# QWERTY6191/projected-lmc

Hardware: AMD Instinct MI355X
Metric: MLL+grad iters/sec, n=8192 16-task LMC (higher is better)
Workload: dtype f32; 1 GPU; C3: ProjectedGPModel+ProjectedLMCmll exact training step (PLMC_fast), n=8192 d=8 p=16 q=8 Matern-5/2 fp32; latents sharded q/N per GPU; n_points=8192, n_dim=8, n_tasks=16, n_latents=8, parallelism=latent-shard x1

## Files before the change

include/plmc.h:

```cpp
#ifndef PLMC_H
#define PLMC_H

#include <stddef.h>
#include <stdint.h>

#ifdef __cplusplus
extern "C" {
#endif

enum { PLMC_RBF = 0, PLMC_MATERN12 = 1, PLMC_MATERN32 = 2, PLMC_MATERN52 = 3, PLMC_SPLINE = 4 };

int         plmc_version(void);
int         plmc_block(void);
int64_t     plmc_pad(int64_t n);
int         plmc_max_dim(void);
const char *plmc_last_error(void);
int64_t     plmc_vd_blocks_for(int64_t n_pad, int64_t lda, int elem_bytes);
int64_t     plmc_vd_blocks(int64_t n_pad, int64_t lda);
int64_t     plmc_vd_blocks_keep(int64_t n_pad, int64_t lda);
int64_t     plmc_split_scales_offset(int64_t n_pad, int64_t lda);
int64_t     plmc_grad_scratch_bytes_for(int64_t n_pad, int q, int elem_bytes);
int64_t     plmc_grad_scratch_bytes(int64_t n_pad, int q);
int64_t     plmc_grad_partials_bytes(int64_t n_pad, int q);

int plmc_assemble_f32(int kind, const float *X, int n, int d, const float *ell, const float *oscale,
                      const float *noise, float *A, int64_t lda, int64_t strideA, int q, void *stream);
int plmc_assemble_f64(int kind, const double *X, int n, int d, const double *ell, const double *oscale,
                      const double *noise, double *A, int64_t lda, int64_t strideA, int q, void *stream);

int plmc_write_rhs_f32(const float *rhs, int nrhs, int n, float *A, int64_t lda, int64_t strideA,
                       int c0, int clear_cols, int q, void *stream);
int plmc_write_rhs_f64(const double *rhs, int nrhs, int n, double *A, int64_t lda, int64_t strideA,
                       int c0, int clear_cols, int q, void *stream);

int plmc_assemble_cross_f32(int kind, const float *X, int n, const float *Xs, int ns, int d,
                            const float *ell, const float *oscale, float *Out, int64_t ldo,
                            int64_t strideO, int64_t col0, int64_t n_rows, int q, void *stream);
int plmc_assemble_cross_f64(int kind, const double *X, int n, const double *Xs, int ns, int d,
                            const double *ell, const double *oscale, double *Out, int64_t ldo,
                            int64_t strideO, int64_t col0, int64_t n_rows, int q, void *stream);

#define PLMC_INFO_CHAIN_ABORT 0x7ffffff0
int plmc_potrf_f32(float *A, int64_t n_pad, int64_t lda, int naug, int64_t strideA, float *Vd,
                   double *logdet, int *info, int with_inverse, int q, void *stream);
int plmc_potrf_f64(double *A, int64_t n_pad, int64_t lda, int naug, int64_t strideA, double *Vd,
                   double *logdet, int *info, int with_inverse, int q, void *stream);
int plmc_potrf_ex_f32(float *A, int64_t n_pad, int64_t lda, int naug, int64_t strideA, float *Vd, double *logdet,
                      int *info, int with_inverse, int q, const float *eig_lo, void *stream);
int plmc_potrf_ex_f64(double *A, int64_t n_pad, int64_t lda, int naug, int64_t strideA, double *Vd, double *logdet,
                      int *info, int with_inverse, int q, const double *eig_lo, void *stream);

int plmc_factorize_ex_f32(int kind, const float *X, int n, int d, const float *ell, const float *oscale, const float *noise,
                          float *A, int64_t n_pad, int64_t lda, int naug, int64_t strideA, float *Vd, double *logdet, int *info,
                          int with_inverse, int q, const float *eig_lo, void *stream);
int plmc_factorize_ex_f64(int kind, const double *X, int n, int d, const double *ell, const double *oscale, const double *noise,
                          double *A, int64_t n_pad, int64_t lda, int naug, int64_t strideA, double *Vd, double *logdet, int *info,
                          int with_inverse, int q, const double *eig_lo, void *stream);

int plmc_potrs_aug_f32(float *A, int64_t n_pad, int64_t lda, int naug, int64_t wcol0, int64_t strideA, float *Vd, int q, void *stream);
int plmc_potrs_aug_f64(double *A, int64_t n_pad, int64_t lda, int naug, int64_t wcol0, int64_t strideA, double *Vd, int q, void *stream);
int plmc_potrs_aug_kept_f32(float *A, int64_t n_pad, int64_t lda, int naug, int64_t wcol0, int64_t strideA, float *Vd, int q,
                            const float *eig_lo, void *stream);
int plmc_potrs_aug_kept_f64(double *A, int64_t n_pad, int64_t lda, int naug, int64_t wcol0, int64_t strideA, double *Vd, int q,
                            const double *eig_lo, void *stream);

int plmc_extract_col_f32(const float *A, int64_t n_pad, int64_t lda, int64_t strideA, int c,
                         float *z, double *quad, int q, void *stream);
int plmc_extract_col_f64(const double *A, int64_t n_pad, int64_t lda, int64_t strideA, int c,
                         double *z, double *quad, int q, void *stream);

int plmc_wt_matvec_f32(const float *W, int64_t n_pad, int64_t ldw, int64_t strideW, const float *z,
                       float *alpha, int q, void *stream);
int plmc_wt_matvec_f64(const double *W, int64_t n_pad, int64_t ldw, int64_t strideW, const double *z,
                       double *alpha, int q, void *stream);

int plmc_gemm_tn_f32(int mode, int M, int N, int K, const float *A, int64_t lda, int64_t strideA, const float *B,
                     int64_t ldb, int64_t strideB, float *C, int64_t ldc, int64_t strideC, int batch, void *stream);
int plmc_gemm_tn_f64(int mode, int M, int N, int K, const double *A, int64_t lda, int64_t strideA, const double *B,
                     int64_t ldb, int64_t strideB, double *C, int64_t ldc, int64_t strideC, int batch, void *stream);
#define PLMC_TRI_A_LOWER 1
#define PLMC_TRI_B_LOWER 2
#define PLMC_TRI_A_UPPER 4
#define PLMC_TRI_C_LOWER 8
#define PLMC_TRI_C_ZERO 16
int plmc_gemm_tn_tri_f32(int mode, int tri, int M, int N, int K, const float *A, int64_t lda, int64_t strideA, const float *B,
                         int64_t ldb, int64_t strideB, float *C, int64_t ldc, int64_t strideC, int batch, void *stream);
int plmc_gemm_tn_tri_f64(int mode, int tri, int M, int N, int K, const double *A, int64_t lda, int64_t strideA, const double *B,
                         int64_t ldb, int64_t strideB, double *C, int64_t ldc, int64_t strideC, int batch, void *stream);

int plmc_posterior_moments_f32(const float *A, int64_t n_pad, int64_t lda, int64_t strideA, int ns, float *mean,
                               float *vsq, int q, void *stream);
int plmc_posterior_moments_f64(const double *A, int64_t n_pad, int64_t lda, int64_t strideA, int ns, double *mean,
                               double *vsq, int q, void *stream);
int plmc_mix_posterior_f32(const float *mean_lat, const float *var_lat, const float *Ht, int q, int ns, int p,
                           double eps, float *mean, float *var, void *stream);
int plmc_mix_posterior_f64(const double *mean_lat, const double *var_lat, const double *Ht, int q, int ns, int p,
                           double eps, double *mean, double *var, void *stream);

int plmc_w_diag_f32(const float *W, int64_t n_pad, int64_t ldw, int64_t strideW, float *kinv_diag, int q,
                    void *stream);
int plmc_w_diag_f64(const double *W, int64_t n_pad, int64_t ldw, int64_t strideW, double *kinv_diag, int q,
                    void *stream);

int plmc_kinv_grad_f32(int kind, const float *W, int64_t n_pad, int64_t ldw, int64_t strideW,
                       const float *alpha, const float *X, int n, int d, const float *ell,
                       const float *oscale, double *grad, float *Kinv, int64_t ldk, int64_t strideK,
                       float *kinv_diag, void *partials, int q, void *stream);
int plmc_kinv_grad_f64(int kind, const double *W, int64_t n_pad, int64_t ldw, int64_t strideW,
                       const double *alpha, const double *X, int n, int d, const double *ell,
                       const double *oscale, double *grad, double *Kinv, int64_t ldk, int64_t strideK,
                       double *kinv_diag, void *partials, int q, void *stream);
int plmc_kinv_grad_ex_f32(int kind, const float *W, int64_t n_pad, int64_t ldw, int64_t strideW,
                          const float *alpha, const float *X, int n, int d, const float *ell,
                          const float *oscale, double *grad, float *Kinv, int64_t ldk, int64_t strideK,
                          float *kinv_diag, void *partials, int q, const float *eig_lo, void *stream);
int plmc_kinv_grad_ex_f64(int kind, const double *W, int64_t n_pad, int64_t ldw, int64_t strideW,
                          const double *alpha, const double *X, int n, int d, const double *ell,
                          const double *oscale, double *grad, double *Kinv, int64_t ldk, int64_t strideK,
                          double *kinv_diag, void *partials, int q, const double *eig_lo, void *stream);
int plmc_kinv_grad_vd_f32(int kind, const float *W, int64_t n_pad, int64_t ldw, int64_t strideW,
                          const float *alpha, const float *X, int n, int d, const float *ell,
                          const float *oscale, double *grad, float *Kinv, int64_t ldk, int64_t strideK,
                          float *kinv_diag, void *partials, int q, const float *eig_lo, const float *Vd, void *stream);
int plmc_kinv_grad_vd_f64(int kind, const double *W, int64_t n_pad, int64_t ldw, int64_t strideW,
                          const double *alpha, const double *X, int n, int d, const double *ell,
                          const double *oscale, double *grad, double *Kinv, int64_t ldk, int64_t strideK,
                          double *kinv_diag, void *partials, int q, const double *eig_lo, const double *Vd, void *stream);

int plmc_max_components(void);
int plmc_assemble_add_f32(int kind, const float *X, int n, int d, int ncomp, const float *ell, const float *oscale,
                          const float *noise, float *A, int64_t lda, int64_t strideA, int q, void *stream);
int plmc_assemble_add_f64(int kind, const double *X, int n, int d, int ncomp, const double *ell, const double *oscale,
                          const double *noise, double *A, int64_t lda, int64_t strideA, int q, void *stream);
int plmc_assemble_cross_add_f32(int kind, const float *X, int n, const float *Xs, int ns, int d, int ncomp,
                                const float *ell, const float *oscale, float *Out, int64_t ldo,
                                int64_t strideO, int64_t col0, int64_t n_rows, int q, void *stream);
int plmc_assemble_cross_add_f64(int kind, const double *X, int n, const double *Xs, int ns, int d, int ncomp,
                                const double *ell, const double *oscale, double *Out, int64_t ldo,
                                int64_t strideO, int64_t col0, int64_t n_rows, int q, void *stream);
int plmc_factorize_add_ex_f32(int kind, const float *X, int n, int d, int ncomp, const float *ell, const float *oscale,
                              const float *noise, float *A, int64_t n_pad, int64_t lda, int naug, int64_t strideA, float *Vd,
                              double *logdet, int *info, int with_inverse, int q, const float *eig_lo, void *stream);
int plmc_factorize_add_ex_f64(int kind, const double *X, int n, int d, int ncomp, const double *ell, const double *oscale,
                              const double *noise, double *A, int64_t n_pad, int64_t lda, int naug, int64_t strideA, double *Vd,
                              double *logdet, int *info, int with_inverse, int q, const double *eig_lo, void *stream);
int plmc_kinv_grad_add_vd_f32(int kind, const float *W, int64_t n_pad, int64_t ldw, int64_t strideW,
                              const float *alpha, const float *X, int n, int d, int ncomp, const float *ell,
                              const float *oscale, double *grad, float *Kinv, int64_t ldk, int64_t strideK,
                              float *kinv_diag, void *partials, int q, const float *eig_lo, const float *Vd, void *stream);
int plmc_kinv_grad_add_vd_f64(int kind, const double *W, int64_t n_pad, int64_t ldw, int64_t strideW,
                              const double *alpha, const double *X, int n, int d, int ncomp, const double *ell,
                              const double *oscale, double *grad, double *Kinv, int64_t ldk, int64_t strideK,
                              double *kinv_diag, void *partials, int q, const double *eig_lo, const double *Vd, void *stream);
int plmc_kernel_vjp_add_f32(int kind, const float *X1, int n1, const float *X2, int n2, int d, int ncomp,
                            const float *ell, const float *oscale, const float *G, int64_t ldg,
                            int64_t strideG, double *gX1, double *gEll, double *gOs, int q, void *stream);
int plmc_kernel_vjp_add_f64(int kind, const double *X1, int n1, const double *X2, int n2, int d, int ncomp,
                            const double *ell, const double *oscale, const double *G, int64_t ldg,
                            int64_t strideG, double *gX1, double *gEll, double *gOs, int q, void *stream);

int plmc_sm_max_mixtures(void);
int plmc_sm_max_dim(void);
int64_t plmc_sm_grad_partials_bytes(int64_t n_pad, int q, int nmix, int elem_bytes);
int plmc_assemble_sm_f32(const float *X, int n, int d, int nmix, const float *scales, const float *means, const float *weights,
                         const float *noise, float *A, int64_t lda, int64_t strideA, int q, void *stream);
int plmc_assemble_sm_f64(const double *X, int n, int d, int nmix, const double *scales, const double *means, const double *weights,
                         const double *noise, double *A, int64_t lda, int64_t strideA, int q, void *stream);
int plmc_assemble_cross_sm_f32(const float *X, int n, const float *Xs, int ns, int d, int nmix, const float *scales, const float *means,
                               const float *weights, float *Out, int64_t ldo, int64_t strideO, int64_t col0, int64_t n_rows, int q,
                               void *stream);
int plmc_assemble_cross_sm_f64(const double *X, int n, const double *Xs, int ns, int d, int nmix, const double *scales, const double *means,
                               const double *weights, double *Out, int64_t ldo, int64_t strideO, int64_t col0, int64_t n_rows, int q,
                               void *stream);
int plmc_factorize_sm_ex_f32(const float *X, int n, int d, int nmix, const float *scales, const float *means, const float *weights,
                             const float *noise, float *A, int64_t n_pad, int64_t lda, int naug, int64_t strideA, float *Vd, double *logdet,
                             int *info, int with_inverse, int q, const float *eig_lo, void *stream);
int plmc_factorize_sm_ex_f64(const double *X, int n, int d, int nmix, const double *scales, const double *means, const double *weights,
                             const double *noise, double *A, int64_t n_pad, int64_t lda, int naug, int64_t strideA, double *Vd, double *logdet,
                             int *info, int with_inverse, int q, const double *eig_lo, void *stream);
int plmc_kinv_grad_sm_vd_f32(const float *W, int64_t n_pad, int64_t ldw, int64_t strideW, const float *alpha, const float *X, int n, int d,
                             int nmix, const float *scales, const float *means, const float *weights, double *grad, float *Kinv, int64_t ldk,
                             int64_t strideK, float *kinv_diag, void *partials, int q, const float *eig_lo, const float *Vd, void *stream);
int plmc_kinv_grad_sm_vd_f64(const double *W, int64_t n_pad, int64_t ldw, int64_t strideW, const double *alpha, const double *X, int n, int d,
                             int nmix, const double *scales, const double *means, const double *weights, double *grad, double *Kinv, int64_t ldk,
                             int64_t strideK, double *kinv_diag, void *partials, int q, const double *eig_lo, const double *Vd, void *stream);

int plmc_per_max_dim(void);
int64_t plmc_per_grad_partials_bytes(int64_t n_pad, int q, int elem_bytes);
int plmc_assemble_per_f32(const float *X, int n, int d, const float *ell, const float *period, const float *oscale, const float *noise,
                          float *A, int64_t lda, int64_t strideA, int q, void *stream);
int plmc_assemble_per_f64(const double *X, int n, int d, const double *ell, const double *period, const double *oscale, const double *noise,
                          double *A, int64_t lda, int64_t strideA, int q, void *stream);
int plmc_assemble_cross_per_f32(const float *X, int n, const float *Xs, int ns, int d, const float *ell, const float *period,
                                const float *oscale, float *Out, int64_t ldo, int64_t strideO, int64_t col0, int64_t n_rows, int q,
                                void *stream);
int plmc_assemble_cross_per_f64(const double *X, int n, const double *Xs, int ns, int d, const double *ell, const double *period,
                                const double *oscale, double *Out, int64_t ldo, int64_t strideO, int64_t col0, int64_t n_rows, int q,
                                void *stream);
int plmc_factorize_per_ex_f32(const float *X, int n, int d, const float *ell, const float *period, const float *oscale, const float *noise,
                              float *A, int64_t n_pad, int64_t lda, int naug, int64_t strideA, float *Vd, double *logdet, int *info,
                              int with_inverse, int q, const float *eig_lo, void *stream);
int plmc_factorize_per_ex_f64(const double *X, int n, int d, const double *ell, const double *period, const double *oscale, const double *noise,
                              double *A, int64_t n_pad, int64_t lda, int naug, int64_t strideA, double *Vd, double *logdet, int *info,
                              int with_inverse, int q, const double *eig_lo, void *stream);
int plmc_kinv_grad_per_vd_f32(const float *W, int64_t n_pad, int64_t ldw, int64_t strideW, const float *alpha, const float *X, int n, int d,
                              const float *ell, const float *period, const float *oscale, double *grad, float *Kinv, int64_t ldk,
                              int64_t strideK, float *kinv_diag, void *partials, int q, const float *eig_lo, const float *Vd, void *stream);
int plmc_kinv_grad_per_vd_f64(const double *W, int64_t n_pad, int64_t ldw, int64_t strideW, const double *alpha, const double *X, int n, int d,
                              const double *ell, const double *period, const double *oscale, double *grad, double *Kinv, int64_t ldk,
                              int64_t strideK, double *kinv_diag, void *partials, int q, const double *eig_lo, const double *Vd, void *stream);

int plmc_comm_unique_id(void *id128);
int plmc_comm_init(const void *id128, int rank, int world);
int plmc_comm_world(void);
int plmc_comm_rank(void);
int plmc_comm_allreduce_sum_f32(float *buf, int64_t count, void *stream);
int plmc_comm_allreduce_sum_f64(double *buf, int64_t count, void *stream);
int plmc_comm_destroy(void);

int64_t plmc_lmc_grad_len(int p, int q, int d);
int64_t plmc_lmc_grad_scratch_bytes(int64_t N_pad, int p, int q, int d);
int plmc_lmc_assemble_f32(int kind, const float *X, int n, int d, int p, int q, const float *ell,
                          const float *oscale, const float *B, const float *Sigma, float *A,
                          int64_t lda, void *stream);
int plmc_lmc_assemble_f64(int kind, const double *X, int n, int d, int p, int q, const double *ell,
                          const double *oscale, const double *B, const double *Sigma, double *A,
                          int64_t lda, void *stream);
int plmc_lmc_cross_f32(int kind, const float *X, int n, const float *Xs, int ns, int d, int p, int q,
                       const float *ell, const float *oscale, const float *B, float *Out, int64_t ldo,
                       int64_t col0, int64_t n_rows, void *stream);
int plmc_lmc_cross_f64(int kind, const double *X, int n, const double *Xs, int ns, int d, int p, int q,
                       const double *ell, const double *oscale, const double *B, double *Out,
                       int64_t ldo, int64_t col0, int64_t n_rows, void *stream);
int plmc_lmc_kinv_grad_f32(int kind, const float *W, int64_t N_pad, int64_t ldw, const float *alpha,
                           const float *X, int n, int d, int p, int q, const float *ell,
                           const float *oscale, const float *B, double *grad, void *partials,
                           void *stream);
int plmc_lmc_kinv_grad_f64(int kind, const double *W, int64_t N_pad, int64_t ldw, const double *alpha,
                           const double *X, int n, int d, int p, int q, const double *ell,
                           const double *oscale, const double *B, double *grad, void *partials,
                           void *stream);

int plmc_kernel_vjp_f32(int kind, const float *X1, int n1, const float *X2, int n2, int d,
                        const float *ell, const float *oscale, const float *G, int64_t ldg,
                        int64_t strideG, double *gX1, double *gEll, double *gOs, int q, void *stream);
int plmc_kernel_vjp_f64(int kind, const double *X1, int n1, const double *X2, int n2, int d,
                        const double *ell, const double *oscale, const double *G, int64_t ldg,
                        int64_t strideG, double *gX1, double *gEll, double *gOs, int q, void *stream);

int plmc_qr_max(void);
int plmc_qr_small_f32(const float *A, int m, int n, int64_t lda, float *Q, int64_t ldq, float *R, int64_t ldr,
                      void *stream);
int plmc_qr_small_f64(const double *A, int m, int n, int64_t lda, double *Q, int64_t ldq, double *R, int64_t ldr,
                      void *stream);

int         plmc_prof_enable(int on);
int         plmc_prof_kernels(void);
const char *plmc_prof_name(int id);
int         plmc_prof_collect(double *ms, int64_t *launches, double *flops, double *bytes);
int         plmc_prof_mfma_rate(int kind, void *sink, int64_t sink_bytes, double *tflops);
int         plmc_dev_reload_knobs(void);

#ifdef __cplusplus
}
#endif
#endif
```

projected-lmc_amd/csrc/api.hip:

```cpp
#include <stdlib.h>
#include <mutex>
#include <vector>

#include "api_common.hpp"
#include "../../include/plmc.h"

namespace plmc {
char *err_buf() {
  static thread_local char buf[256] = {0};
  return buf;
}

static const char *kProfNames[PK_COUNT] = {"k_assemble", "k_write_rhs", "k_assemble_cross", "k_diag",   "k_panel",
                                           "k_trail",    "k_wdiag",     "k_trtri_row",      "k_extract_col",
                                           "k_wt_matvec", "k_kinv_grad", "k_reduce_grad", "k_kernel_vjp",
                                           "sweep_total", "k_trail_row", "k_trail_head", "k_gpanel", "k_split_w", "k_posterior_moments"};
struct ProfRec { int id; hipEvent_t a, b; double flops, bytes; };
static unsigned g_prof_mask = 0;
static std::vector<ProfRec> g_recs;
static std::vector<hipEvent_t> g_free;

static hipEvent_t get_event() {
  if (!g_free.empty()) { hipEvent_t e = g_free.back(); g_free.pop_back(); return e; }
  hipEvent_t e;
  if (hipEventCreate(&e) != hipSuccess) return nullptr;
  return e;
}

static std::recursive_mutex g_api_mutex;
void api_lock() { g_api_mutex.lock(); }
void api_unlock() { g_api_mutex.unlock(); }

static Knobs g_knobs;
static bool g_knobs_loaded = false;
static void load_knobs() {
  const char *h = getenv("PLMC_HALF_TILES"), *g = getenv("PLMC_GRP");
  g_knobs.half_tiles = h ? (atoi(h) == 1 ? 1e30 : (double)atoi(h)) : 640.0;
  g_knobs.grp = g ? atoi(g) : 0;
  g_knobs.serial = getenv("PLMC_SERIAL") && atoi(getenv("PLMC_SERIAL")) != 0;
  g_knobs.bulk_lds = getenv("PLMC_BULK_LDS") ? atoi(getenv("PLMC_BULK_LDS")) : -1;
  g_knobs.split = getenv("PLMC_SPLIT") ? atoi(getenv("PLMC_SPLIT")) : 2;
  if (g_knobs.split != 0 && g_knobs.split != 3) g_knobs.split = 2;
  g_knobs.bulk_streams = getenv("PLMC_BULK_STREAMS") ? atoi(getenv("PLMC_BULK_STREAMS")) : 2;
  g_knobs.chain = getenv("PLMC_CHAIN") ? atoi(getenv("PLMC_CHAIN")) : 1;
  g_knobs.chain_nw = getenv("PLMC_CHAIN_NW") ? atoi(getenv("PLMC_CHAIN_NW")) : 0;
  g_knobs.chain_edge = getenv("PLMC_CHAIN_EDGE") ? atoi(getenv("PLMC_CHAIN_EDGE")) : 0;
  g_knobs_loaded = true;
}
const Knobs &knobs() {
  if (!g_knobs_loaded) {
    std::lock_guard<std::recursive_mutex> lk(g_api_mutex);
    if (!g_knobs_loaded) load_knobs();
  }
  return g_knobs;
}

constexpr int SWEEP_CTX = 2;
struct SweepCtx {
  hipStream_t caller = nullptr;
  bool used = false;
  unsigned long long stamp = 0;
  hipStream_t side[2] = {nullptr, nullptr};
  hipEvent_t ev[16] = {nullptr};
};
static SweepCtx g_ctx[64][SWEEP_CTX];
static unsigned long long g_stamp = 0;
static thread_local int t_ctx = 0;
static SweepCtx *cur_ctx() {
  int dev = 0;
  if (hipGetDevice(&dev) != hipSuccess || dev < 0 || dev >= 64) return nullptr;
  return &g_ctx[dev][t_ctx];
}
hipStream_t side_stream(int which) {
  SweepCtx *c = cur_ctx();
  if (!c || which < 0 || which > 1) return nullptr;
  if (!c->side[which]) {
    int lo = 0, hi = 0;
    (void)hipDeviceGetStreamPriorityRange(&lo, &hi);
    if (hipStreamCreateWithPriority(&c->side[which], hipStreamNonBlocking, hi) != hipSuccess) c->side[which] = nullptr;
  }
  return c->side[which];
}
hipEvent_t sync_event(int idx) {
  SweepCtx *c = cur_ctx();
  if (!c) return nullptr;
  hipEvent_t &e = c->ev[idx & 15];
  if (!e && hipEventCreateWithFlags(&e, hipEventDisableTiming) != hipSuccess) e = nullptr;
  return e;
}
void bind_sweep_ctx(hipStream_t caller, int e_prev_idx) {
  int dev = 0;
  if (hipGetDevice(&dev) != hipSuccess || dev < 0 || dev >= 64) { t_ctx = 0; return; }
  SweepCtx *set = g_ctx[dev];
  int pick = -1;
  for (int i = 0; i < SWEEP_CTX; ++i)
    if (set[i].used && set[i].caller == caller) pick = i;
  if (pick < 0) {
    for (int i = 0; i < SWEEP_CTX && pick < 0; ++i)
      if (!set[i].used) pick = i;
    if (pick < 0) {
      pick = 0;
      for (int i = 1; i < SWEEP_CTX; ++i)
        if (set[i].stamp < set[pick].stamp) pick = i;
      if (set[pick].ev[e_prev_idx & 15]) (void)hipStreamWaitEvent(caller, set[pick].ev[e_prev_idx & 15], 0);
    }
    set[pick].caller = caller;
    set[pick].used = true;
  }
  set[pick].stamp = ++g_stamp;
  t_ctx = pick;
}

template <typename T>
__global__ __launch_bounds__(NTHREADS) void k_mfma_rate(T *sink, int iters) {
  using Tr = Traits<T>;
  typename Tr::acc_t acc[16];
#pragma unroll
  for (int i = 0; i < 16; ++i)
#pragma unroll
    for (int r = 0; r < 4; ++r) acc[i][r] = T(0);
  T a[4], b[4];
#pragma unroll
  for (int i = 0; i < 4; ++i) { a[i] = T(1) + T(threadIdx.x & 7) * T(1e-3) + T(i); b[i] = T(0.5) - T(i) * T(1e-3); }
#pragma unroll 1
  for (int it = 0; it < iters; ++it) {
#pragma unroll
    for (int i = 0; i < 16; ++i) acc[i] = Tr::mfma(a[i >> 2], b[i & 3], acc[i]);
  }
  T s = T(0);
#pragma unroll
  for (int i = 0; i < 16; ++i) s += acc[i][0] + acc[i][1] + acc[i][2] + acc[i][3];
  sink[(size_t)blockIdx.x * NTHREADS + threadIdx.x] = s;
}

typedef __bf16 rate_bf16x8 __attribute__((ext_vector_type(8)));
__global__ __launch_bounds__(NTHREADS) void k_mfma_rate_bf16(float *sink, int iters) {
  f32x4 acc[16];
#pragma unroll
  for (int i = 0; i < 16; ++i)
#pragma unroll
    for (int r = 0; r < 4; ++r) acc[i][r] = 0.f;
  rate_bf16x8 a[4], b[4];
#pragma unroll
  for (int i = 0; i < 4; ++i)
#pragma unroll
    for (int j = 0; j < 8; ++j) { a[i][j] = (__bf16)(1.0f + 0.01f * (float)((threadIdx.x + j) & 7) + (float)i); b[i][j] = (__bf16)(0.5f - 0.01f * (float)(i + j)); }
#pragma unroll 1
  for (int it = 0; it < iters; ++it) {
#pragma unroll
    for (int i = 0; i < 16; ++i) acc[i] = __builtin_amdgcn_mfma_f32_16x16x32_bf16(a[i >> 2], b[i & 3], acc[i], 0, 0, 0);
  }
  float s = 0.f;
#pragma unroll
  for (int i = 0; i < 16; ++i) s += acc[i][0] + acc[i][1] + acc[i][2] + acc[i][3];
  sink[(size_t)blockIdx.x * NTHREADS + threadIdx.x] = s;
}

template <typename T, bool BF16 = false> static int mfma_rate_impl(void *sink, int64_t sink_bytes, double *tflops) {
  int dev = 0;
  hipDeviceProp_t prop;
  if (hipGetDevice(&dev) != hipSuccess || hipGetDeviceProperties(&prop, dev) != hipSuccess) return fail("plmc_prof_mfma_rate", "no device");
  const int grid = 4 * prop.multiProcessorCount, iters = 4000;
  if (!sink || !tflops || sink_bytes < (int64_t)grid * NTHREADS * (int64_t)sizeof(T)) return fail("plmc_prof_mfma_rate", "sink too small");
  hipEvent_t e0 = nullptr, e1 = nullptr;
  if (hipEventCreate(&e0) != hipSuccess || hipEventCreate(&e1) != hipSuccess) return fail("plmc_prof_mfma_rate", "event");
  double best = 0.0;
  for (int rep = 0; rep < 3; ++rep) {
    (void)hipEventRecord(e0, nullptr);
    if (BF16) hipLaunchKernelGGL(k_mfma_rate_bf16, dim3(grid), dim3(NTHREADS), 0, nullptr, (float *)sink, iters);
    else hipLaunchKernelGGL(k_mfma_rate<T>, dim3(grid), dim3(NTHREADS), 0, nullptr, (T *)sink, iters);
    (void)hipEventRecord(e1, nullptr);
    float ms = 0.f;
    if (hipEventSynchronize(e1) != hipSuccess || hipEventElapsedTime(&ms, e0, e1) != hipSuccess) break;
    const double fl = (double)grid * (NTHREADS / 64) * (double)iters * 16.0 * 2.0 * 16 * 16 * (BF16 ? 32 : 4);
    if (ms > 0.f && fl / (ms * 1e-3) / 1e12 > best) best = fl / (ms * 1e-3) / 1e12;
  }
  (void)hipEventDestroy(e0);
  (void)hipEventDestroy(e1);
  *tflops = best;
  return launch_status("plmc_prof_mfma_rate");
}

ProfScope::ProfScope(int id, hipStream_t st, double flops, double bytes) : idx_(-1), st_(st) {
  api_lock();
  if (!((g_prof_mask >> id) & 1u) || g_recs.size() >= (1u << 20)) return;
  ProfRec r{id, get_event(), get_event(), flops, bytes};
  if (!r.a || !r.b) return;
  (void)hipEventRecord(r.a, st);
  g_recs.push_back(r);
  idx_ = (long)g_recs.size() - 1;
}
ProfScope::~ProfScope() {
  if (idx_ >= 0) (void)hipEventRecord(g_recs[idx_].b, st_);
  api_unlock();
}
}

extern "C" {
int plmc_version(void) { return 4; }
int plmc_block(void) { return plmc::NB; }
int64_t plmc_pad(int64_t n) { return (n + plmc::NB - 1) / plmc::NB * plmc::NB; }
int plmc_max_dim(void) { return plmc::MAX_DIM; }
const char *plmc_last_error(void) { return plmc::err_buf(); }

int plmc_prof_enable(int on) {
  std::lock_guard<std::recursive_mutex> lk(plmc::g_api_mutex);
  const unsigned prev = plmc::g_prof_mask, all = (1u << plmc::PK_COUNT) - 1u;
  plmc::g_prof_mask = on == 0 ? 0u : (on == 1 ? all : ((unsigned)on >> 1) & all);
  return prev == 0 ? 0 : (prev == all ? 1 : (int)(prev << 1));
}
int plmc_prof_mfma_rate(int kind, void *sink, int64_t sink_bytes, double *tflops) {
  if (kind == 2) return plmc::mfma_rate_impl<float, true>(sink, sink_bytes, tflops);
  return kind ? plmc::mfma_rate_impl<double>(sink, sink_bytes, tflops) : plmc::mfma_rate_impl<float>(sink, sink_bytes, tflops);
}
int plmc_dev_reload_knobs(void) {
  std::lock_guard<std::recursive_mutex> lk(plmc::g_api_mutex);
  plmc::load_knobs();
  return 0;
}
int plmc_prof_kernels(void) { return plmc::PK_COUNT; }
const char *plmc_prof_name(int id) { return (id >= 0 && id < plmc::PK_COUNT) ? plmc::kProfNames[id] : ""; }
int plmc_prof_collect(double *ms, int64_t *launches, double *flops, double *bytes) {
  using namespace plmc;
  std::lock_guard<std::recursive_mutex> lk(g_api_mutex);
  for (int i = 0; i < PK_COUNT; ++i) { ms[i] = 0; launches[i] = 0; flops[i] = 0; bytes[i] = 0; }
  for (auto &r : g_recs) {
    float t = 0.f;
    if (hipEventSynchronize(r.b) == hipSuccess && hipEventElapsedTime(&t, r.a, r.b) == hipSuccess) {
      ms[r.id] += t; launches[r.id] += 1; flops[r.id] += r.flops; bytes[r.id] += r.bytes;
    }
    g_free.push_back(r.a);
    g_free.push_back(r.b);
  }
  g_recs.clear();
  return 0;
}
}
```

projected-lmc_amd/csrc/api_common.hpp:

```cpp
#pragma once
#include <hip/hip_runtime.h>
#include <stdint.h>
#include <stdio.h>
#include <string.h>

#include "gemm_core.hpp"
#include "covariance.hpp"

namespace plmc {

constexpr int MAX_DIM = 32;
constexpr int MAX_COMP = 4;
constexpr int SM_MAX_MIX = 8;
constexpr int SM_MAX_DIM = 8;
constexpr int PER_MAX_DIM = 8;

char *err_buf();

inline int fail(const char *fn, const char *msg) {
  snprintf(err_buf(), 256, "%s: %s", fn, msg);
  return -1;
}

inline int launch_status(const char *fn) {
  hipError_t e = hipGetLastError();
  if (e != hipSuccess) {
    snprintf(err_buf(), 256, "%s: HIP launch failed: %s", fn, hipGetErrorString(e));
    return -2;
  }
  return 0;
}

#define PLMC_REQUIRE(cond, msg) \
  do { if (!(cond)) return plmc::fail(__func__, msg); } while (0)

enum ProfKernel { PK_ASSEMBLE, PK_WRITE_RHS, PK_CROSS, PK_DIAG, PK_PANEL, PK_TRAIL, PK_WDIAG, PK_TRTRI, PK_EXTRACT,
                  PK_WTMV, PK_KINV_GRAD, PK_REDUCE, PK_VJP, PK_SWEEP, PK_TRAIL_ROW, PK_TRAIL_HEAD, PK_GPANEL, PK_SPLIT, PK_POST, PK_COUNT };

struct ProfScope {
  ProfScope(int id, hipStream_t st, double flops, double bytes);
  ~ProfScope();
  long idx_;
  hipStream_t st_;
};

struct Knobs {
  double half_tiles;
  int grp;
  bool serial;
  int bulk_lds;
  int split;
  int bulk_streams;
  int chain;
  int chain_edge;
  int chain_nw;
};
const Knobs &knobs();

enum CovFamily { COV_PLAIN, COV_ADD, COV_SM, COV_PER };
struct CovTable {
  CovFamily family;
  int kind, d, ncomp;
  const void *ell, *second, *oscale;
  static CovTable plain(int kind, int d, const void *ell, const void *oscale) { return {COV_PLAIN, kind, d, 1, ell, nullptr, oscale}; }
  static CovTable add(int kind, int d, int ncomp, const void *ell, const void *oscale) { return {COV_ADD, kind, d, ncomp, ell, nullptr, oscale}; }
  static CovTable sm(int d, int nmix, const void *scales, const void *means, const void *weights) { return {COV_SM, 0, d, nmix, scales, means, weights}; }
  static CovTable per(int d, const void *ell, const void *period, const void *oscale) { return {COV_PER, 0, d, 1, ell, period, oscale}; }
  const char *check() const {
    if (family == COV_ADD) {
      if (kind < 0 || kind > K_MATERN52) return "additive kernels take the stationary kinds only (no spline kernel)";
      if (ncomp < 1 || ncomp > MAX_COMP) return "need 1 <= components <= plmc_max_components()";
    } else if (family == COV_SM) {
      if (ncomp < 1 || ncomp > SM_MAX_MIX) return "need 1 <= mixtures <= plmc_sm_max_mixtures()";
      if (d <= 0 || d > SM_MAX_DIM) return "need 0 < d <= plmc_sm_max_dim()";
    } else if (family == COV_PER) {
      if (d <= 0 || d > PER_MAX_DIM) return "need 0 < d <= plmc_per_max_dim()";
    }
    return (family == COV_SM || family == COV_PER) && !second ? "null pointer" : nullptr;
  }
  CovFamily route() const { return family == COV_ADD && ncomp == 1 ? COV_PLAIN : family; }
  int partials_rows() const { return family == COV_ADD || family == COV_SM ? ncomp : 1; }
};
#define PLMC_REQUIRE_TABLE(t) \
  do { if (const char *why_ = (t).check()) return plmc::fail(__func__, why_); } while (0)

struct AssembleJob {
  CovTable table;
  int n;
  const void *X, *noise;
};
int assemble_rows(const AssembleJob &job, int elem_bytes, void *A, int64_t lda, int64_t strideA, int q, int ib0, int nrows, void *stream,
                  int ncols = -1, int skip = 0);

hipStream_t side_stream(int which = 0);
hipEvent_t sync_event(int idx);
void bind_sweep_ctx(hipStream_t caller, int e_prev_idx);

inline bool aligned16(const void *p) { return (reinterpret_cast<uintptr_t>(p) & 15) == 0; }

}
```

projected-lmc_amd/csrc/kinv_epilogue.inc:

```
  const int lane = tid & 63, wave = tid >> 6;
  const int wm = wave >> 1, wn = wave & 1;
  const T *el = ell + (int64_t)lat * d;
  const T os = oscale ? oscale[lat] : T(1);
  T g_noise = T(0), g_os = T(0);
  auto wave_sum = [&](double v) {
#pragma unroll
    for (int o = 32; o > 0; o >>= 1) v += __shfl_down(v, o, 64);
    return v;
  };
  double *red;

  if constexpr (DCAP <= 8) {
    typedef GradLds<DCAP> L;
    T g[DCAP];
#pragma unroll
    for (int k = 0; k < DCAP; ++k) g[k] = T(0);
    static_assert(L::END <= tile_smem_elems<T>(), "gradient epilogue LDS plan");
    for (int e = tid; e < NB * DCAP; e += NTHREADS) {
      const int r = e / DCAP, k = e % DCAP;
      const int gi = ib * NB + r, gj = jb * NB + r;
      const T inv = k < d ? T(1) / el[k] : T(0);
      smem[L::UI + r * L::LDI + k] = (k < d && gi < n) ? X[(int64_t)gi * d + k] * inv : T(0);
      smem[L::UJ + r * L::LDI + k] = (k < d && gj < n) ? X[(int64_t)gj * d + k] * inv : T(0);
    }
    if (tid < NB) {
      smem[L::AI + tid] = live ? alpha[(int64_t)lat * n_pad + ib * NB + tid] : T(0);
      smem[L::AJ + tid] = live ? alpha[(int64_t)lat * n_pad + jb * NB + tid] : T(0);
    }
    __syncthreads();
    const bool interior = ib < jb && (jb + 1) * NB <= n && !Kinv && !kinv_diag;
#define PLMC_GRAD_TILE(KIND, INT) \
  grad_tile_small<T, DCAP, KIND, INT>(acc, smem, tid, os, ib, jb, n, lat, n_pad, Kinv, ldk, strideK, kinv_diag, g, g_noise, g_os)
    if (interior) {
      if (kind == K_RBF) PLMC_GRAD_TILE(K_RBF, true);
      else if (kind == K_MATERN12) PLMC_GRAD_TILE(K_MATERN12, true);
      else if (kind == K_MATERN32) PLMC_GRAD_TILE(K_MATERN32, true);
      else if (kind == K_MATERN52) PLMC_GRAD_TILE(K_MATERN52, true);
      else PLMC_GRAD_TILE(K_SPLINE, false);
    } else {
      if (kind == K_RBF) PLMC_GRAD_TILE(K_RBF, false);
      else if (kind == K_MATERN12) PLMC_GRAD_TILE(K_MATERN12, false);
      else if (kind == K_MATERN32) PLMC_GRAD_TILE(K_MATERN32, false);
      else if (kind == K_MATERN52) PLMC_GRAD_TILE(K_MATERN52, false);
      else PLMC_GRAD_TILE(K_SPLINE, false);
    }
#undef PLMC_GRAD_TILE
    __syncthreads();
    red = reinterpret_cast<double *>(smem);
#pragma unroll
    for (int k = 0; k < DCAP; ++k) {
      const double s = wave_sum((double)g[k]);
      if (lane == 0) red[wave * GP + k] = s;
    }
  } else {
  constexpr bool KEEP = PLMC_KINV_KEEP;
  constexpr int GH = KEEP ? DCAP : 8;
  constexpr int KD = KEEP ? DCAP : 1;
  const int ldu = d + 1;
  T *ui = smem;
  T *uj = ui + NB * ldu;
  T *ai = uj + NB * ldu;
  T *aj = ai + NB;
  red = reinterpret_cast<double *>(aj + NB);
  static_assert((2 * NB * (MAX_DIM + 1) + 2 * NB) * sizeof(T) + 4 * GP * sizeof(double) <= tile_smem_elems<T>() * sizeof(T),
                "general gradient epilogue LDS plan");
  for (int e = tid; e < NB * d; e += NTHREADS) {
    int r = e / d, k = e % d;
    int gi = ib * NB + r, gj = jb * NB + r;
    T inv = T(1) / el[k];
    ui[r * ldu + k] = gi < n ? X[(int64_t)gi * d + k] * inv : T(0);
    uj[r * ldu + k] = gj < n ? X[(int64_t)gj * d + k] * inv : T(0);
  }
  if (tid < NB) {
    ai[tid] = live ? alpha[(int64_t)lat * n_pad + ib * NB + tid] : T(0);
    aj[tid] = live ? alpha[(int64_t)lat * n_pad + jb * NB + tid] : T(0);
  }
  __syncthreads();
#pragma unroll 1
  for (int k0 = 0; k0 < DCAP; k0 += GH) {
    T g[GH];
#pragma unroll
    for (int k = 0; k < GH; ++k) g[k] = T(0);
    const bool first = k0 == 0;
    if (first || (k0 < d && !SPLINE)) {
#pragma unroll
      for (int mt = 0; mt < 4; ++mt) {
#pragma unroll 1
        for (int r = 0; r < 4; ++r) {
          const int row = tile_row<T>(wm, mt, lane, r);
          const int gi = ib * NB + row;
          T xi[KD];
          const T *uir = ui + row * ldu;
          if constexpr (KEEP) {
#pragma unroll
            for (int k = 0; k < DCAP; ++k) xi[k] = k < d ? uir[k] : T(0);
          }
          const T a_i = ai[row];
#pragma unroll
          for (int nt = 0; nt < 4; ++nt) {
            const int col = tile_col(wn, nt, lane);
            const int gj = jb * NB + col;
            const auto &av = acc.v[mt][nt];
            const T kin = r == 0 ? av[0] : (r == 1 ? av[1] : (r == 2 ? av[2] : av[3]));
            if (first) {
              if (Kinv && gj >= gi) Kinv[(int64_t)lat * strideK + (int64_t)gi * ldk + gj] = kin;
              if (kinv_diag && gi == gj) kinv_diag[(int64_t)lat * n_pad + gi] = kin;
            }
            if (gi < n && gj < n && gj >= gi) {
              const T wij = a_i * aj[col] - kin;
              const T *ujc = uj + col * ldu;
              T df2[KD];
              T r2 = T(0);
              if constexpr (KEEP) {
#pragma unroll
                for (int k = 0; k < DCAP; ++k) {
                  T df = k < d ? xi[k] - ujc[k] : T(0);
                  df2[k] = df * df;
                  r2 += df2[k];
                }
              } else {
#pragma unroll 4
                for (int k = 0; k < d; ++k) { const T df = uir[k] - ujc[k]; r2 += df * df; }
              }
              T val, base;
              if constexpr (SPLINE) {
                val = T(1);
                if constexpr (KEEP) {
#pragma unroll
                  for (int k = 0; k < DCAP; ++k) val *= k < d ? spline_factor(xi[k], ujc[k]) : T(1);
                } else {
#pragma unroll 4
                  for (int k = 0; k < d; ++k) val *= spline_factor(uir[k], ujc[k]);
                }
                base = T(0);
              } else {
                kern_value_base_fast(kind, r2, val, base);
              }
              if (gi == gj) {
                if (first) { g_noise += wij; g_os += wij * val; }
              } else {
                const T c = T(2) * wij * os * base;
                if constexpr (KEEP) {
#pragma unroll
                  for (int k = 0; k < DCAP; ++k) g[k] += c * df2[k];
                } else if constexpr (!SPLINE) {
#pragma unroll
                  for (int k = 0; k < GH; ++k) {
                    const T df = k0 + k < d ? uir[k0 + k] - ujc[k0 + k] : T(0);
                    g[k] += c * df * df;
                  }
                }
                if (first) g_os += T(2) * wij * val;
              }
            }
          }
        }
      }
    }
#pragma unroll
    for (int k = 0; k < GH; ++k) {
      const double s = wave_sum((double)g[k]);
      if (lane == 0) red[wave * GP + k0 + k] = s;
    }
  }
  }

  {
    double s = wave_sum((double)g_noise);
    if (lane == 0) red[wave * GP + MAX_DIM] = s;
    s = wave_sum((double)g_os);
    if (lane == 0) red[wave * GP + MAX_DIM + 1] = s;
  }
  __syncthreads();
  double *out = partials + (((int64_t)lat * m + ib) * m + jb) * GP;
  if (live && tid < GP) {
    const bool used = tid < DCAP || tid >= MAX_DIM;
    out[tid] = used ? red[tid] + red[GP + tid] + red[2 * GP + tid] + red[3 * GP + tid] : 0.0;
  }
```

projected-lmc_amd/csrc/potri_grad.hip:

```cpp
#include <stdlib.h>
#include "api_common.hpp"
#include "covariance.hpp"
#include "bf3_engine.hpp"
#include "vd_layout.hpp"
#include "../../include/plmc.h"

namespace plmc {

constexpr int GP = MAX_DIM + 2;

template <int DCAP> struct GradLds {
  static constexpr int LDI = DCAP + 4;
  static constexpr int UI = 0, UJ = UI + NB * LDI, AI = UJ + NB * LDI, AJ = AI + NB, ACCS = AJ + NB, END = ACCS + 4 * NTHREADS * 4;
};

template <typename T, int DCAP, int KIND, bool INTERIOR>
__device__ __forceinline__ void grad_tile_small(const Acc<T> &acc, T *smem, const int tid, T os, int ib, int jb, int n, int lat, int64_t n_pad,
                                                T *Kinv, int64_t ldk, int64_t strideK, T *kinv_diag, T (&g)[DCAP],
                                                T &g_noise, T &g_os) {
  typedef Pair<T> T2;
  typedef GradLds<DCAP> L;
  constexpr int NP = DCAP / 2;
  const int lane = tid & 63, wave = tid >> 6;
  const int wm = wave >> 1, wn = wave & 1;
  T2 g2[NP];
#pragma unroll
  for (int j = 0; j < NP; ++j) g2[j] = T2{T(0), T(0)};
  T gos = T(0), gnz = T(0);
  T *accs = smem + L::ACCS + tid * 4;
#pragma unroll 1
  for (int mt = 0; mt < 4; ++mt) {
#define PLMC_PARK(M)                                                                                    \
  _Pragma("unroll") for (int nt = 0; nt < 4; ++nt) _Pragma("unroll") for (int r = 0; r < 4; ++r)         \
      accs[nt * NTHREADS * 4 + r] = acc.v[M][nt][r];
    if (mt == 0) { PLMC_PARK(0) } else if (mt == 1) { PLMC_PARK(1) } else if (mt == 2) { PLMC_PARK(2) } else { PLMC_PARK(3) }
#undef PLMC_PARK
#pragma unroll 1
    for (int nt = 0; nt < 4; ++nt) {
      const int col = tile_col(wn, nt, lane);
      const T *ujc = smem + L::UJ + col * L::LDI;
      T2 u2[NP];
#pragma unroll
      for (int j = 0; j < NP; ++j) u2[j] = *reinterpret_cast<const T2 *>(ujc + 2 * j);
      const T a_j = smem[L::AJ + col];
      const int gj = jb * NB + col;
#pragma unroll 1
      for (int r = 0; r < 4; ++r) {
        const int row = tile_row<T>(wm, mt, lane, r);
        const T kin = accs[nt * NTHREADS * 4 + r];
        const T *uir = smem + L::UI + row * L::LDI;
        T2 df[NP];
        T2 r2p = {T(0), T(0)};
#pragma unroll
        for (int j = 0; j < NP; ++j) {
          df[j] = *reinterpret_cast<const T2 *>(uir + 2 * j) - u2[j];
          r2p += df[j] * df[j];
        }
        T val, base;
        if constexpr (KIND == K_SPLINE) {
          val = T(1);
#pragma unroll
          for (int j = 0; j < NP; ++j) {
            const T2 xr = *reinterpret_cast<const T2 *>(uir + 2 * j);
            val *= spline_factor(xr.x, u2[j].x) * spline_factor(xr.y, u2[j].y);
          }
          base = T(0);
        } else {
          kern_value_base_fast(KIND, r2p.x + r2p.y, val, base);
        }
        T w = smem[L::AI + row] * a_j - kin;
        if (!INTERIOR) {
          const int gi = ib * NB + row;
          if (Kinv && gj >= gi) Kinv[(int64_t)lat * strideK + (int64_t)gi * ldk + gj] = kin;
          if (kinv_diag && gi == gj) kinv_diag[(int64_t)lat * n_pad + gi] = kin;
          const bool live = gi < n && gj < n && gj >= gi;
          if (live && gi == gj) gnz += w;
          w = live ? (gj > gi ? T(2) * w : w) : T(0);
        }
        gos += w * val;
        const T c = w * base;
#pragma unroll
        for (int j = 0; j < NP; ++j) g2[j] += (c * df[j]) * df[j];
      }
    }
  }
  const T sc = INTERIOR ? T(2) * os : os;
#pragma unroll
  for (int j = 0; j < NP; ++j) {
    g[2 * j] += sc * g2[j].x;
    g[2 * j + 1] += sc * g2[j].y;
  }
  g_os += INTERIOR ? T(2) * gos : gos;
  g_noise += gnz;
}

template <typename T, int DCAP> constexpr int KG_MIN_WAVES = sizeof(T) == 8 ? 2 : (DCAP <= 8 ? 4 : (DCAP <= 16 ? 2 : 1));

template <typename T, int DCAP, bool SPLINE>
__device__ __forceinline__ void kinv_tile_epilogue(const Acc<T> &acc, T *smem, const int tid, const bool live, int kind, int ib, int jb, int lat,
                                                   int m, int64_t n_pad, const T *__restrict__ alpha, const T *__restrict__ X, int n, int d,
                                                   const T *__restrict__ ell, const T *__restrict__ oscale, T *Kinv, int64_t ldk,
                                                   int64_t strideK, T *kinv_diag, double *__restrict__ partials) {
  if (!live) { n = 0; Kinv = nullptr; kinv_diag = nullptr; }
#define PLMC_KINV_KEEP (DCAP <= 16)
#include "kinv_epilogue.inc"
#undef PLMC_KINV_KEEP
}

#define PLMC_KINV_TILE_PRODUCT                                                                                                                 \
  const int m = (int)(n_pad / NB);                                                                                                             \
  const int lat = (int)blockIdx.x % nlat;                                                                                                      \
  int ib, jb;                                                                                                                                  \
  tri_decode((int)blockIdx.x / nlat, ib, jb);                                                                                                  \
  __shared__ __align__(16) T smem[tile_smem_elems<T>()];                                                                                       \
  const T *Wl = W + (int64_t)lat * strideW + (int64_t)jb * NB * ldw;                                                                           \
  Acc<T> acc;                                                                                                                                  \
  acc.zero();                                                                                                                                  \
  tile_mainloop<T, false, true>(acc, Wl + (int64_t)ib * NB, ldw, Wl + (int64_t)jb * NB, ldw, (int)(n_pad - (int64_t)jb * NB), smem)

template <typename T, int DCAP, bool SPLINE = false>
__global__ __launch_bounds__(NTHREADS, (KG_MIN_WAVES<T, DCAP>)) void k_kinv_grad(int kind, const T *__restrict__ W, int64_t n_pad, int64_t ldw,
                                                         int64_t strideW, const T *__restrict__ alpha,
                                                         const T *__restrict__ X, int n, int d,
                                                         const T *__restrict__ ell, const T *__restrict__ oscale,
                                                         T *Kinv, int64_t ldk, int64_t strideK, T *kinv_diag,
                                                         double *__restrict__ partials, int nlat) {
  PLMC_KINV_TILE_PRODUCT;
  const int tid = threadIdx.x;
  constexpr bool live = true;
#define PLMC_KINV_KEEP (sizeof(T) == 4)
#include "kinv_epilogue.inc"
#undef PLMC_KINV_KEEP
}

#define PLMC_KINV_BF3_TILE_PRODUCT                                                                                                             \
  constexpr int LDS_BYTES = b3_lds_bytes<S>() > 2 * tile_smem_elems<float>() * (int)sizeof(float) ? b3_lds_bytes<S>() : 2 * tile_smem_elems<float>() * (int)sizeof(float); \
  __shared__ __align__(16) unsigned char lds[LDS_BYTES];                                                                                       \
  const int m = (int)(n_pad / NB);                                                                                                             \
  const int SJ = (m + 7) / 8, NSB = SJ * (SJ + 1) / 2;                                                                                         \
  const int w = blockIdx.x, xcd = w & 7, slot = w >> 3;                                                                                        \
  const int gb = xcd + 8 * (slot >> 5), in = slot & 31;                                                                                        \
  if (gb >= nlat * NSB) return;                                                                                                                \
  const int lat = gb / NSB;                                                                                                                    \
  int sa, sj;                                                                                                                                  \
  tri_decode(gb - lat * NSB, sa, sj);                                                                                                          \
  const int ibm = 2 * (4 * sa + (in >> 3)), jb = 8 * sj + (in & 7);                                                                            \
  if (jb >= m || ibm > jb) return;                                                                                                             \
  Acc<float> acc0, acc1;                                                                                                                       \
  acc0.zero();                                                                                                                                 \
  acc1.zero();                                                                                                                                 \
  if (ws_stride > 1) {                                                                                                                         \
    ws_stride = (int64_t)wscale[VD_W_TAG + 1] * NB * NB;                                                                                       \
    wp_lat_stride = 2 * ws_stride;                                                                                                             \
  }                                                                                                                                            \
  const unsigned short *Pl = Wp + (int64_t)lat * wp_lat_stride + b3_index<S>((int64_t)jb * NB, 0, 0, n_pad);                                   \
  b3_mainloop<S, 2, 0, B3NoPre, true>(acc0, acc1, Pl + (int64_t)ibm * NB * 8, n_pad, Pl + (int64_t)jb * NB * 8, n_pad, (int)(n_pad - (int64_t)jb * NB), lds); \
  float ws = wscale[(int64_t)lat * ws_stride];                                                                                                 \
  if (ws_stride > 1 && wscale[(int64_t)lat * ws_stride + VD_W_TAG] != (float)S::NPL) ws = __builtin_nanf("");                                  \
  b3_combine<S>(acc0, acc1, 1.0f / (ws * ws));                                                                                                 \
  const int half = __builtin_amdgcn_readfirstlane((int)threadIdx.x >> 8);                                                                      \
  const int ib = ibm + half

template <class S, int DCAP, bool SPLINE = false>
__global__ __launch_bounds__(B3_NT, 2) void k_kinv_grad_bf3(int kind, int64_t n_pad, const float *__restrict__ alpha, const float *__restrict__ X, int n,
                                                            int d, const float *__restrict__ ell, const float *__restrict__ oscale, float *Kinv,
                                                            int64_t ldk, int64_t strideK, float *kinv_diag, double *__restrict__ partials, int nlat,
                                                            const unsigned short *__restrict__ Wp, const float *__restrict__ wscale,
                                                            int64_t wp_lat_stride, int64_t ws_stride) {
  PLMC_KINV_BF3_TILE_PRODUCT;
  kinv_tile_epilogue<float, DCAP, SPLINE>(acc0, reinterpret_cast<float *>(lds) + half * tile_smem_elems<float>(), (int)threadIdx.x & 255, ib <= jb, kind,
                                          ib, jb, lat, m, n_pad, alpha, X, n, d, ell, oscale, Kinv, ldk, strideK, kinv_diag, partials);
}


template <typename T, CovFamily F, int DC>
__device__ __forceinline__ void kinv_tile_epilogue_add(const Acc<T> &acc, T *smem, const int tid, const bool live, int kind, int ncomp, int ib, int jb,
                                                       int lat, int m, int64_t n_pad, const T *__restrict__ alpha, const T *__restrict__ X, int n, int d,
                                                       const T *__restrict__ ell, const T *__restrict__ oscale, T *Kinv, int64_t ldk,
                                                       int64_t strideK, T *kinv_diag, double *__restrict__ partials, const T *__restrict__ means) {
  if (!live) { n = 0; Kinv = nullptr; kinv_diag = nullptr; }
#include "kinv_epilogue_table.inc"
}

template <typename T, CovFamily F, int DC = 0>
__global__ __launch_bounds__(NTHREADS, (sizeof(T) == 8 && (F == COV_SM || (F == COV_PER && DC > 1)) ? 1 : 2)) void k_kinv_grad_add(int kind, int ncomp, const T *__restrict__ W, int64_t n_pad, int64_t ldw,
                                                                int64_t strideW, const T *__restrict__ alpha, const T *__restrict__ X, int n, int d,
                                                                const T *__restrict__ ell, const T *__restrict__ oscale, T *Kinv, int64_t ldk,
                                                                int64_t strideK, T *kinv_diag, double *__restrict__ partials, int nlat,
                                                                const T *__restrict__ means) {
  PLMC_KINV_TILE_PRODUCT;
  const int tid = threadIdx.x;
  constexpr bool live = true;
#include "kinv_epilogue_table.inc"
}

template <class S, CovFamily F, int DC = 0>
__global__ __launch_bounds__(B3_NT, 2) void k_kinv_grad_add_bf3(int kind, int ncomp, int64_t n_pad, const float *__restrict__ alpha,
                                                                const float *__restrict__ X, int n, int d, const float *__restrict__ ell,
                                                                const float *__restrict__ oscale, float *Kinv, int64_t ldk, int64_t strideK,
                                                                float *kinv_diag, double *__restrict__ partials, int nlat,
                                                                const unsigned short *__restrict__ Wp, const float *__restrict__ wscale,
                                                                int64_t wp_lat_stride, int64_t ws_stride, const float *__restrict__ means) {
  PLMC_KINV_BF3_TILE_PRODUCT;
  kinv_tile_epilogue_add<float, F, DC>(acc0, reinterpret_cast<float *>(lds) + half * tile_smem_elems<float>(), (int)threadIdx.x & 255, ib <= jb, kind, ncomp,
                                       ib, jb, lat, m, n_pad, alpha, X, n, d, ell, oscale, Kinv, ldk, strideK, kinv_diag, partials, means);
}

constexpr int RED_NT = 1024;
#define PLMC_REDUCE_TILES(tstride, row0)                                                      \
  __shared__ double red[RED_NT];                                                              \
  const int lat = blockIdx.x;                                                                 \
  const int ntile = m * m;                                                                    \
  const int slot = threadIdx.x % GP;                                                          \
  const int grp = threadIdx.x / GP;                                                           \
  constexpr int NG = RED_NT / GP;                                                             \
  double s[4] = {0.0, 0.0, 0.0, 0.0};                                                         \
  if (grp < NG) {                                                                             \
    const double *base = partials + (int64_t)lat * ntile * (tstride) + (row0) + slot;         \
    for (int t0 = grp; t0 < ntile; t0 += 4 * NG) {                                            \
      _Pragma("unroll") for (int u = 0; u < 4; ++u) {                                         \
        const int t = t0 + u * NG;                                                            \
        if (t < ntile) {                                                                      \
          const int ib = t / m, jb = t - ib * m;                                              \
          if (jb >= ib) s[u] += base[(int64_t)t * (tstride)];                                 \
        }                                                                                     \
      }                                                                                       \
    }                                                                                         \
  }                                                                                           \
  red[threadIdx.x] = (s[0] + s[1]) + (s[2] + s[3]);                                           \
  __syncthreads()
__device__ __forceinline__ double reduce_slot_total(const double *red) {
  double tot = 0.0;
  for (int gq = 0; gq < RED_NT / GP; ++gq) tot += red[gq * GP + threadIdx.x];
  return tot;
}

template <typename T>
__global__ __launch_bounds__(RED_NT) void k_reduce_grad(const double *__restrict__ partials, int m, int d,
                                                        const T *__restrict__ ell, double *__restrict__ grad) {
  PLMC_REDUCE_TILES(GP, 0);
  if (threadIdx.x < GP) {
    const double tot = reduce_slot_total(red);
    const int k = threadIdx.x;
    if (k < d) grad[(int64_t)lat * (d + 2) + k] = 0.5 * tot / (double)ell[(int64_t)lat * d + k];
    else if (k == MAX_DIM) grad[(int64_t)lat * (d + 2) + d] = 0.5 * tot;
    else if (k == MAX_DIM + 1) grad[(int64_t)lat * (d + 2) + d + 1] = 0.5 * tot;
  }
}

template <typename T, bool SM = false>
__global__ __launch_bounds__(RED_NT) void k_reduce_grad_add(const double *__restrict__ partials, int m, int d, int ncomp,
                                                            const T *__restrict__ ell, double *__restrict__ grad) {
  const int g = blockIdx.y;
  const int64_t tstride = (int64_t)ncomp * GP;
  PLMC_REDUCE_TILES(tstride, (int64_t)g * GP);
  if (threadIdx.x < GP) {
    const double tot = reduce_slot_total(red);
    const int k = threadIdx.x;
    if constexpr (SM) {
      double *gl = grad + (int64_t)lat * (ncomp * (2 * d + 1) + 1);
      if (k < d) gl[g * d + k] = -2.0 * SM_2PI2 * 0.5 * tot;
      else if (k >= SM_MAX_DIM && k < SM_MAX_DIM + d) gl[(ncomp + g) * d + k - SM_MAX_DIM] = -SM_2PI * 0.5 * tot;
      else if (k == MAX_DIM && g == 0) gl[2 * ncomp * d] = 0.5 * tot;
      else if (k == MAX_DIM + 1) gl[2 * ncomp * d + 1 + g] = 0.5 * tot;
      return;
    }
    double *gl = grad + (int64_t)lat * (ncomp * (d + 1) + 1);
    if (k < d) gl[g * d + k] = 0.5 * tot / (double)ell[((int64_t)lat * ncomp + g) * d + k];
    else if (k == MAX_DIM && g == 0) gl[ncomp * d] = 0.5 * tot;
    else if (k == MAX_DIM + 1) gl[ncomp * d + 1 + g] = 0.5 * tot;
  }
}

template <typename T>
__global__ __launch_bounds__(RED_NT) void k_reduce_grad_per(const double *__restrict__ partials, int m, int d, const T *__restrict__ ell,
                                                            const T *__restrict__ period, double *__restrict__ grad) {
  PLMC_REDUCE_TILES(GP, 0);
  if (threadIdx.x < GP) {
    const double tot = reduce_slot_total(red);
    const int k = threadIdx.x;
    double *gl = grad + (int64_t)lat * (2 * d + 2);
    if (k < d) {
      const double l = (double)ell[(int64_t)lat * d + k];
      gl[k] = 0.5 * tot / (l * l);
    } else if (k >= PER_MAX_DIM && k < PER_MAX_DIM + d) {
      const int kk = k - PER_MAX_DIM;
      const double l = (double)ell[(int64_t)lat * d + kk], p = (double)period[(int64_t)lat * d + kk];
      gl[d + kk] = 0.5 * tot * SM_2PI / (l * p * p);
    } else if (k == MAX_DIM) gl[2 * d] = 0.5 * tot;
    else if (k == MAX_DIM + 1) gl[2 * d + 1] = 0.5 * tot;
  }
}

template <class S>
__global__ __launch_bounds__(NTHREADS) void k_split_w(const float *__restrict__ W, int64_t n_pad, int64_t ldw, int64_t strideW,
                                                      unsigned short *__restrict__ Wp, const float *__restrict__ wscale) {
  const int cb = blockIdx.x, lb = blockIdx.y, lat = blockIdx.z;
  if (cb > lb) return;
  b3_split_block<S, false>(W + (int64_t)lat * strideW + (int64_t)lb * NB * ldw + (int64_t)cb * NB, ldw,
                           Wp + (int64_t)lat * b3_elems<S>(n_pad, n_pad) + b3_index<S>((int64_t)lb * NB, 0, (int64_t)cb * NB, n_pad), n_pad, wscale[lat],
                           nullptr, 0, threadIdx.x);
}
template <class S>
__global__ void k_w_scale(const float *__restrict__ eig_lo, float *__restrict__ wscale, int q, int padded) {
  const int lat = threadIdx.x;
  if (lat >= q) return;
  if constexpr (S::NPL == 3) wscale[lat] = 1.0f;
  else {
    float lam = fmaxf(eig_lo[lat], 1e-30f);
    if (padded) lam = fminf(lam, 1.0f);
    wscale[lat] = b3_scale_for(1.0f / sqrtf(lam));
  }
}

template <typename T, class S>
int kinv_grad_impl(const CovTable &table, const T *W, int64_t n_pad, int64_t ldw, int64_t strideW, const T *alpha, const T *X, int n, double *grad,
                   T *Kinv, int64_t ldk, int64_t strideK, T *kinv_diag, void *partials, int q, const float *eig_lo, void *stream,
                   const float *Vd = nullptr, int64_t lda_vd = 0) {
  PLMC_REQUIRE_TABLE(table);
  const CovFamily family = table.route();
  const int kind = table.kind, d = table.d, ncomp = table.ncomp, rows = table.partials_rows();
  const T *ell = (const T *)table.ell, *oscale = (const T *)table.oscale, *second = (const T *)table.second;
  PLMC_REQUIRE(kind >= 0 && kind <= 4, "unknown kernel kind");
  PLMC_REQUIRE(W && alpha && X && ell && grad && partials, "null pointer");
  PLMC_REQUIRE(n_pad > 0 && n_pad % NB == 0 && ldw % NB == 0 && n <= n_pad && n > n_pad - NB, "n_pad must be plmc_pad(n)");
  PLMC_REQUIRE(d > 0 && d <= MAX_DIM && q > 0, "need 0<d<=plmc_max_dim(), q>0");
  PLMC_REQUIRE(!Kinv || (ldk >= n_pad), "ldk too small");
  PLMC_REQUIRE(aligned16(W), "unaligned W");
  hipStream_t st = (hipStream_t)stream;
  const int m = (int)(n_pad / NB);
  double *part = reinterpret_cast<double *>(partials);
  const double np = (double)n_pad;
  if constexpr (!std::is_void<S>::value) {
    PLMC_REQUIRE(q <= 1024, "too many latents for one scale launch");
    const unsigned short *wp = nullptr;
    const float *wsc = nullptr;
    int64_t wp_lat = b3_elems<S>(n_pad, n_pad), ws_lat = 1;
    if (!(Vd && vd_w_planes(Vd, n_pad, lda_vd, &wp, &wp_lat, &wsc, &ws_lat))) {
      PLMC_REQUIRE(family != COV_PER && family != COV_SM,
                   family == COV_PER ? "the periodic gradient call takes the planes of W from the sweep's Vd (factorise with the inverse factor)"
                                     : "the spectral-mixture gradient call takes the planes of W from the sweep's Vd (factorise with the inverse factor)");
      char *pb = reinterpret_cast<char *>(partials) + (int64_t)m * m * q * rows * GP * (int64_t)sizeof(double);
      unsigned short *wpo = reinterpret_cast<unsigned short *>(pb);
      float *wsco = reinterpret_cast<float *>(pb + (int64_t)q * b3_elems<SplitB3>(n_pad, n_pad) * 2);
      hipLaunchKernelGGL((k_w_scale<S>), dim3(1), dim3(q < 64 ? 64 : ((q + 63) / 64) * 64), 0, st, eig_lo, wsco, q, (int)(n < n_pad));
      ProfScope ps(PK_SPLIT, st, 0.0, (double)q * np * np / 2 * (4 + 2 * S::NPL));
      hipLaunchKernelGGL((k_split_w<S>), dim3(m, m, q), dim3(NTHREADS), 0, st, (const float *)W, n_pad, ldw, strideW, wpo, (const float *)wsco);
      wp = wpo;
      wsc = wsco;
      wp_lat = b3_elems<S>(n_pad, n_pad);
      ws_lat = 1;
    }
    const int SJ = (m + 7) / 8, NSB = SJ * (SJ + 1) / 2;
    const dim3 gridb(8 * ((q * NSB + 7) / 8) * 32);
#define PLMC_LAUNCH_KB(DC, SP) \
  hipLaunchKernelGGL((k_kinv_grad_bf3<S, DC, SP>), gridb, dim3(B3_NT), 0, st, kind, n_pad, alpha, X, n, d, ell, oscale, Kinv, ldk, strideK, kinv_diag, \
                     part, q, wp, wsc, wp_lat, ws_lat)
#define PLMC_LAUNCH_TB(F, DC) \
  hipLaunchKernelGGL((k_kinv_grad_add_bf3<S, F, DC>), gridb, dim3(B3_NT), 0, st, kind, ncomp, n_pad, alpha, X, n, d, ell, oscale, Kinv, ldk, strideK, \
                     kinv_diag, part, q, wp, wsc, wp_lat, ws_lat, (const float *)second)
    ProfScope ps(PK_KINV_GRAD, st, q * np * np * np / 3.0, q * (np * np / 2) * sizeof(T));
    switch (family) {
      case COV_PER: PLMC_LAUNCH_TB(COV_PER, 1); break;
      case COV_SM: PLMC_LAUNCH_TB(COV_SM, 1); break;
      case COV_ADD: PLMC_LAUNCH_TB(COV_ADD, 0); break;
      case COV_PLAIN:
        if (d <= 4) PLMC_LAUNCH_KB(4, false);
        else if (d <= 8) PLMC_LAUNCH_KB(8, false);
        else if (d <= 16) { if (kind == K_SPLINE) PLMC_LAUNCH_KB(16, true); else PLMC_LAUNCH_KB(16, false); }
        else { if (kind == K_SPLINE) PLMC_LAUNCH_KB(32, true); else PLMC_LAUNCH_KB(32, false); }
    }
#undef PLMC_LAUNCH_TB
#undef PLMC_LAUNCH_KB
  } else {
    const dim3 grid(q * (m * (m + 1) / 2)), block(NTHREADS);
#define PLMC_LAUNCH_KG(DC, SP)                                                                                       \
  hipLaunchKernelGGL((k_kinv_grad<T, DC, SP>), grid, block, 0, st, kind, W, n_pad, ldw, strideW, alpha, X, n, d, ell, \
                     oscale, Kinv, ldk, strideK, kinv_diag, part, q)
#define PLMC_LAUNCH_TG(F, DC) \
  hipLaunchKernelGGL((k_kinv_grad_add<T, F, DC>), grid, block, 0, st, kind, ncomp, W, n_pad, ldw, strideW, alpha, X, n, d, ell, oscale, Kinv, ldk, \
                     strideK, kinv_diag, part, q, second)
    ProfScope ps(PK_KINV_GRAD, st, q * np * np * np / 3.0, q * (np * np / 2) * sizeof(T));
    switch (family) {
      case COV_PER: if (d == 1) PLMC_LAUNCH_TG(COV_PER, 1); else if (d <= 4) PLMC_LAUNCH_TG(COV_PER, 4); else PLMC_LAUNCH_TG(COV_PER, 8); break;
      case COV_SM: if (d == 1) PLMC_LAUNCH_TG(COV_SM, 1); else if (d <= 4) PLMC_LAUNCH_TG(COV_SM, 4); else PLMC_LAUNCH_TG(COV_SM, 8); break;
      case COV_ADD: PLMC_LAUNCH_TG(COV_ADD, 0); break;
      case COV_PLAIN:
        if (d <= 4) PLMC_LAUNCH_KG(4, false);
        else if (d <= 8) PLMC_LAUNCH_KG(8, false);
        else if (d <= 16) { if (kind == K_SPLINE) PLMC_LAUNCH_KG(16, true); else PLMC_LAUNCH_KG(16, false); }
        else { if (kind == K_SPLINE) PLMC_LAUNCH_KG(32, true); else PLMC_LAUNCH_KG(32, false); }
    }
#undef PLMC_LAUNCH_TG
#undef PLMC_LAUNCH_KG
  }
  {
    ProfScope ps(PK_REDUCE, st, 0.0, (double)m * m * q * rows * GP * sizeof(double) / 2);
    switch (family) {
      case COV_PER: hipLaunchKernelGGL(k_reduce_grad_per<T>, dim3(q), dim3(RED_NT), 0, st, part, m, d, ell, second, grad); break;
      case COV_SM: hipLaunchKernelGGL((k_reduce_grad_add<T, true>), dim3(q, ncomp), dim3(RED_NT), 0, st, part, m, d, ncomp, ell, grad); break;
      case COV_ADD: hipLaunchKernelGGL((k_reduce_grad_add<T, false>), dim3(q, ncomp), dim3(RED_NT), 0, st, part, m, d, ncomp, ell, grad); break;
      case COV_PLAIN: hipLaunchKernelGGL(k_reduce_grad<T>, dim3(q), dim3(RED_NT), 0, st, part, m, d, ell, grad);
    }
  }
  return launch_status(__func__);
}

}

extern "C" {
int64_t plmc_grad_scratch_bytes_for(int64_t n_pad, int q, int elem_bytes) {
  int64_t m = n_pad / plmc::NB;
  const int64_t planes = elem_bytes == 4 ? (int64_t)q * plmc::b3_elems<plmc::SplitB3>(n_pad, n_pad) * 2 + 4096 : 0;
  return m * m * (int64_t)q * plmc::GP * (int64_t)sizeof(double) + planes;
}
int64_t plmc_grad_scratch_bytes(int64_t n_pad, int q) { return plmc_grad_scratch_bytes_for(n_pad, q, 4); }
int64_t plmc_grad_partials_bytes(int64_t n_pad, int q) {
  const int64_t m = n_pad / plmc::NB;
  return m * m * (int64_t)q * plmc::GP * (int64_t)sizeof(double);
}
static int kinv_grad_f32_any(const plmc::CovTable &table, const float *W, int64_t n_pad, int64_t ldw, int64_t strideW, const float *alpha,
                             const float *X, int n, double *grad, float *Kinv, int64_t ldk, int64_t strideK, float *kinv_diag, void *partials, int q,
                             const float *eig_lo, void *stream, const float *Vd = nullptr) {
  const int split = plmc::knobs().split;
  if (split == 0 || ((table.family == plmc::COV_SM || table.family == plmc::COV_PER) && table.d > 1))
    return plmc::kinv_grad_impl<float, void>(table, W, n_pad, ldw, strideW, alpha, X, n, grad, Kinv, ldk, strideK, kinv_diag, partials, q, nullptr, stream);
  if (split == 2 && eig_lo)
    return plmc::kinv_grad_impl<float, plmc::SplitH2>(table, W, n_pad, ldw, strideW, alpha, X, n, grad, Kinv, ldk, strideK, kinv_diag, partials, q, eig_lo,
                                                      stream, Vd, ldw);
  return plmc::kinv_grad_impl<float, plmc::SplitB3>(table, W, n_pad, ldw, strideW, alpha, X, n, grad, Kinv, ldk, strideK, kinv_diag, partials, q, nullptr,
                                                    stream, Vd, ldw);
}
static int kinv_grad_f64(const plmc::CovTable &table, const double *W, int64_t n_pad, int64_t ldw, int64_t strideW, const double *alpha,
                         const double *X, int n, double *grad, double *Kinv, int64_t ldk, int64_t strideK, double *kinv_diag, void *partials, int q,
                         void *stream) {
  return plmc::kinv_grad_impl<double, void>(table, W, n_pad, ldw, strideW, alpha, X, n, grad, Kinv, ldk, strideK, kinv_diag, partials, q, nullptr, stream);
}
using plmc::CovTable;
int plmc_kinv_grad_f32(int kind, const float *W, int64_t n_pad, int64_t ldw, int64_t strideW, const float *alpha,
                       const float *X, int n, int d, const float *ell, const float *oscale, double *grad,
                       float *Kinv, int64_t ldk, int64_t strideK, float *kinv_diag, void *partials, int q,
                       void *stream) {
  return kinv_grad_f32_any(CovTable::plain(kind, d, ell, oscale), W, n_pad, ldw, strideW, alpha, X, n, grad, Kinv, ldk, strideK, kinv_diag, partials, q,
                           nullptr, stream);
}
int plmc_kinv_grad_ex_f32(int kind, const float *W, int64_t n_pad, int64_t ldw, int64_t strideW, const float *alpha,
                          const float *X, int n, int d, const float *ell, const float *oscale, double *grad,
                          float *Kinv, int64_t ldk, int64_t strideK, float *kinv_diag, void *partials, int q,
                          const float *eig_lo, void *stream) {
  return kinv_grad_f32_any(CovTable::plain(kind, d, ell, oscale), W, n_pad, ldw, strideW, alpha, X, n, grad, Kinv, ldk, strideK, kinv_diag, partials, q,
                           eig_lo, stream);
}
int plmc_kinv_grad_vd_f32(int kind, const float *W, int64_t n_pad, int64_t ldw, int64_t strideW, const float *alpha,
                          const float *X, int n, int d, const float *ell, const float *oscale, double *grad,
                          float *Kinv, int64_t ldk, int64_t strideK, float *kinv_diag, void *partials, int q,
                          const float *eig_lo, const float *Vd, void *stream) {
  return kinv_grad_f32_any(CovTable::plain(kind, d, ell, oscale), W, n_pad, ldw, strideW, alpha, X, n, grad, Kinv, ldk, strideK, kinv_diag, partials, q,
                           eig_lo, stream, Vd);
}
int plmc_kinv_grad_vd_f64(int kind, const double *W, int64_t n_pad, int64_t ldw, int64_t strideW, const double *alpha,
                          const double *X, int n, int d, const double *ell, const double *oscale, double *grad,
                          double *Kinv, int64_t ldk, int64_t strideK, double *kinv_diag, void *partials, int q,
                          const double *eig_lo, const double *Vd, void *stream) {
  (void)eig_lo;
  (void)Vd;
  return kinv_grad_f64(CovTable::plain(kind, d, ell, oscale), W, n_pad, ldw, strideW, alpha, X, n, grad, Kinv, ldk, strideK, kinv_diag, partials, q, stream);
}
int plmc_kinv_grad_add_vd_f32(int kind, const float *W, int64_t n_pad, int64_t ldw, int64_t strideW, const float *alpha,
                              const float *X, int n, int d, int ncomp, const float *ell, const float *oscale, double *grad,
                              float *Kinv, int64_t ldk, int64_t strideK, float *kinv_diag, void *partials, int q,
                              const float *eig_lo, const float *Vd, void *stream) {
  return kinv_grad_f32_any(CovTable::add(kind, d, ncomp, ell, oscale), W, n_pad, ldw, strideW, alpha, X, n, grad, Kinv, ldk, strideK, kinv_diag, partials,
                           q, eig_lo, stream, Vd);
}
int plmc_kinv_grad_add_vd_f64(int kind, const double *W, int64_t n_pad, int64_t ldw, int64_t strideW, const double *alpha,
                              const double *X, int n, int d, int ncomp, const double *ell, const double *oscale, double *grad,
                              double *Kinv, int64_t ldk, int64_t strideK, double *kinv_diag, void *partials, int q,
                              const double *eig_lo, const double *Vd, void *stream) {
  (void)eig_lo;
  (void)Vd;
  return kinv_grad_f64(CovTable::add(kind, d, ncomp, ell, oscale), W, n_pad, ldw, strideW, alpha, X, n, grad, Kinv, ldk, strideK, kinv_diag, partials, q,
                       stream);
}
int64_t plmc_sm_grad_partials_bytes(int64_t n_pad, int q, int nmix, int elem_bytes) {
  (void)elem_bytes;
  return plmc_grad_partials_bytes(n_pad, q * nmix);
}
int plmc_kinv_grad_sm_vd_f32(const float *W, int64_t n_pad, int64_t ldw, int64_t strideW, const float *alpha, const float *X, int n, int d,
                             int nmix, const float *scales, const float *means, const float *weights, double *grad, float *Kinv, int64_t ldk,
                             int64_t strideK, float *kinv_diag, void *partials, int q, const float *eig_lo, const float *Vd, void *stream) {
  return kinv_grad_f32_any(CovTable::sm(d, nmix, scales, means, weights), W, n_pad, ldw, strideW, alpha, X, n, grad, Kinv, ldk, strideK, kinv_diag,
                           partials, q, eig_lo, stream, Vd);
}
int plmc_kinv_grad_sm_vd_f64(const double *W, int64_t n_pad, int64_t ldw, int64_t strideW, const double *alpha, const double *X, int n, int d,
                             int nmix, const double *scales, const double *means, const double *weights, double *grad, double *Kinv, int64_t ldk,
                             int64_t strideK, double *kinv_diag, void *partials, int q, const double *eig_lo, const double *Vd, void *stream) {
  (void)eig_lo;
  (void)Vd;
  return kinv_grad_f64(CovTable::sm(d, nmix, scales, means, weights), W, n_pad, ldw, strideW, alpha, X, n, grad, Kinv, ldk, strideK, kinv_diag, partials,
                       q, stream);
}
int64_t plmc_per_grad_partials_bytes(int64_t n_pad, int q, int elem_bytes) {
  (void)elem_bytes;
  return plmc_grad_partials_bytes(n_pad, q);
}
int plmc_kinv_grad_per_vd_f32(const float *W, int64_t n_pad, int64_t ldw, int64_t strideW, const float *alpha, const float *X, int n, int d,
                              const float *ell, const float *period, const float *oscale, double *grad, float *Kinv, int64_t ldk,
                              int64_t strideK, float *kinv_diag, void *partials, int q, const float *eig_lo, const float *Vd, void *stream) {
  return kinv_grad_f32_any(CovTable::per(d, ell, period, oscale), W, n_pad, ldw, strideW, alpha, X, n, grad, Kinv, ldk, strideK, kinv_diag, partials, q,
                           eig_lo, stream, Vd);
}
int plmc_kinv_grad_per_vd_f64(const double *W, int64_t n_pad, int64_t ldw, int64_t strideW, const double *alpha, const double *X, int n, int d,
                              const double *ell, const double *period, const double *oscale, double *grad, double *Kinv, int64_t ldk,
                              int64_t strideK, double *kinv_diag, void *partials, int q, const double *eig_lo, const double *Vd, void *stream) {
  (void)eig_lo;
  (void)Vd;
  return kinv_grad_f64(CovTable::per(d, ell, period, oscale), W, n_pad, ldw, strideW, alpha, X, n, grad, Kinv, ldk, strideK, kinv_diag, partials, q,
                       stream);
}
int plmc_kinv_grad_f64(int kind, const double *W, int64_t n_pad, int64_t ldw, int64_t strideW, const double *alpha,
                       const double *X, int n, int d, const double *ell, const double *oscale, double *grad,
                       double *Kinv, int64_t ldk, int64_t strideK, double *kinv_diag, void *partials, int q,
                       void *stream) {
  return kinv_grad_f64(CovTable::plain(kind, d, ell, oscale), W, n_pad, ldw, strideW, alpha, X, n, grad, Kinv, ldk, strideK, kinv_diag, partials, q, stream);
}
int plmc_kinv_grad_ex_f64(int kind, const double *W, int64_t n_pad, int64_t ldw, int64_t strideW, const double *alpha,
                          const double *X, int n, int d, const double *ell, const double *oscale, double *grad,
                          double *Kinv, int64_t ldk, int64_t strideK, double *kinv_diag, void *partials, int q,
                          const double *eig_lo, void *stream) {
  (void)eig_lo;
  return kinv_grad_f64(CovTable::plain(kind, d, ell, oscale), W, n_pad, ldw, strideW, alpha, X, n, grad, Kinv, ldk, strideK, kinv_diag, partials, q, stream);
}
}
```

projected-lmc_amd/projectedlmc/_engine.py:

```python
import math
import os

import torch

from . import _hip
from . import settings
from ._pivot import PivotCheck, deferred_pivot_checks, walk

LOG2PI = math.log(2.0 * math.pi)


class Workspace:

    def __init__(self, n, q, naug, dtype, device, with_inverse=True, keep_planes=False, ncomp=1, sm=False, per=False):
        L = _hip.lib()
        self.n, self.q, self.naug, self.dtype, self.device = n, q, naug, dtype, device
        self.ncomp = ncomp
        self.with_inverse = bool(with_inverse)
        self.keep_planes = bool(keep_planes) and self.with_inverse and dtype == torch.float32
        self.NB = L.cdll.plmc_block()
        self.n_pad = int(L.cdll.plmc_pad(n))
        self.naug_pad = int(L.cdll.plmc_pad(naug)) if naug > 0 else 0
        self.wcol0 = self.n_pad + self.naug_pad
        self.lda = self.wcol0 + (self.n_pad if with_inverse else 0)
        if (self.lda // self.NB) % 2 == 0:
            self.lda += self.NB
        self.strideA = self.n_pad * self.lda
        esz = torch.empty((), dtype=dtype).element_size()
        vd_blocks = L.cdll.plmc_vd_blocks_keep(self.n_pad, self.lda) if self.keep_planes else L.cdll.plmc_vd_blocks_for(self.n_pad, self.lda, esz)
        self.Vd = torch.empty(q, int(vd_blocks), self.NB, self.NB, dtype=dtype, device=device)
        self.m = self.n_pad // self.NB
        self.A = torch.empty(q, self.n_pad, self.lda, dtype=dtype, device=device)
        self.logdet = torch.empty(q, dtype=torch.float64, device=device)
        self.quad = torch.empty(q, dtype=torch.float64, device=device)
        self.info = torch.empty(q, dtype=torch.int32, device=device)
        self.z = torch.empty(q, self.n_pad, dtype=dtype, device=device)
        self.W = self.alpha = self.partials = None
        if with_inverse:
            self.W = self.A[:, :, self.wcol0:self.wcol0 + self.n_pad]
            self.ldw, self.strideW = self.lda, self.strideA
            self.alpha = torch.empty(q, self.n_pad, dtype=dtype, device=device)
            nbytes = int(L.cdll.plmc_sm_grad_partials_bytes(self.n_pad, q, ncomp, esz) if sm
                         else L.cdll.plmc_per_grad_partials_bytes(self.n_pad, q, esz) if per
                         else L.cdll.plmc_grad_partials_bytes(self.n_pad, q * ncomp))
            self.partials = torch.empty(nbytes // 8, dtype=torch.float64, device=device)


_ws_cache = {}


def _release(ws):
    pending = getattr(ws, "pending", None)
    if pending is not None:
        torch.cuda.current_stream(ws.device).wait_event(pending)
        ws.pending = None


def _drop_all():
    for ws in _ws_cache.values():
        _release(ws)
    _ws_cache.clear()


def get_workspace(n, q, naug, dtype, device, need_grad, ncomp=1, sm=False, per=False):
    ncomp = ncomp if need_grad else 1
    sm = bool(sm) and bool(need_grad)
    per = bool(per) and bool(need_grad)
    key = (n, q, naug, dtype, device.index, bool(need_grad), ncomp, sm, per)
    ws = _ws_cache.get(key)
    if ws is None:
        if len(_ws_cache) > 3:
            _drop_all()
        ws = Workspace(n, q, naug, dtype, device, need_grad, ncomp=ncomp, sm=sm, per=per)
        _ws_cache[key] = ws
    _release(ws)
    return ws


_grad_streams = {}


def grad_stream(device):
    if os.environ.get("PLMC_GRAD_STREAM", "1") == "0":
        return None
    s = _grad_streams.get(device.index)
    if s is None:
        s = _grad_streams[device.index] = torch.cuda.Stream(device)
    return s


def free_workspaces():
    _drop_all()


def _contig(t, dtype=None):
    if t is None:
        return None
    t = t.detach()
    if dtype is not None and t.dtype != dtype:
        t = t.to(dtype)
    return t.contiguous()


PER = "periodic"
_PER = {"plmc_assemble": "plmc_assemble_per", "plmc_assemble_cross": "plmc_assemble_cross_per",
        "plmc_factorize_ex": "plmc_factorize_per_ex", "plmc_kinv_grad_vd": "plmc_kinv_grad_per_vd"}
_SM = {"plmc_assemble": "plmc_assemble_sm", "plmc_assemble_cross": "plmc_assemble_cross_sm",
       "plmc_factorize_ex": "plmc_factorize_sm_ex", "plmc_kinv_grad_vd": "plmc_kinv_grad_sm_vd"}
_ADD = {"plmc_assemble": "plmc_assemble_add", "plmc_assemble_cross": "plmc_assemble_cross_add",
        "plmc_factorize_ex": "plmc_factorize_add_ex", "plmc_kinv_grad_vd": "plmc_kinv_grad_add_vd",
        "plmc_kernel_vjp": "plmc_kernel_vjp_add"}


def is_sm(ell):
    return ell.dim() == 4


def n_components(ell, kind=None):
    if kind == PER:
        return 1
    return ell.shape[2] if ell.dim() == 4 else (ell.shape[1] if ell.dim() == 3 else 1)


def kind_code(kind):
    return None if kind == "sm" else (PER if kind == PER else _hip.KIND[kind])


def grad_table_width(ell, kind=None):
    return ell[0].numel() + 1 + n_components(ell, kind)


def _check_kernel_shape(L, ell, kind=None):
    d = ell.shape[-1]
    if d > L.cdll.plmc_max_dim():
        raise ValueError("input dimension %d exceeds plmc_max_dim()=%d" % (d, L.cdll.plmc_max_dim()))
    if kind == PER:
        if ell.dim() != 3 or ell.shape[1] != 2:
            raise ValueError("a periodic kernel's table is (q, 2, d) = [lengthscales | periods]")
        if d > L.cdll.plmc_per_max_dim():
            raise ValueError("periodic kernel on %d dimensions exceeds plmc_per_max_dim()=%d" % (d, L.cdll.plmc_per_max_dim()))
    elif is_sm(ell):
        if d > L.cdll.plmc_sm_max_dim() or n_components(ell) > L.cdll.plmc_sm_max_mixtures():
            raise ValueError("spectral mixture with %d components on %d dimensions exceeds plmc_sm_max_mixtures()=%d / plmc_sm_max_dim()=%d"
                             % (n_components(ell), d, L.cdll.plmc_sm_max_mixtures(), L.cdll.plmc_sm_max_dim()))
    elif n_components(ell) > L.cdll.plmc_max_components():
        raise ValueError("%d additive components exceed plmc_max_components()=%d" % (n_components(ell), L.cdll.plmc_max_components()))


def _kernel_call(L, base, dt, head, ell, tail, stream=None):
    if isinstance(head[0], str) and head[0] == PER:
        rows = getattr(ell, "_per_rows", None)
        if rows is None:
            rows = ell._per_rows = (ell[:, 0].contiguous(), ell[:, 1].contiguous())
        if stream is not None:
            rows[0].record_stream(stream)
            rows[1].record_stream(stream)
        L.call(_PER[base], dt, *head[1:], _hip.ptr(rows[0]), _hip.ptr(rows[1]), *tail)
    elif ell.dim() == 4:
        planes = getattr(ell, "_sm_planes", None)
        if planes is None:
            planes = ell._sm_planes = (ell[:, 0].contiguous(), ell[:, 1].contiguous())
        scales, means = planes
        if stream is not None:
            scales.record_stream(stream)
            means.record_stream(stream)
        L.call(_SM[base], dt, *head[1:], ell.shape[2], _hip.ptr(scales), _hip.ptr(means), *tail)
    elif ell.dim() == 3:
        L.call(_ADD[base], dt, *head, ell.shape[1], _hip.ptr(ell), *tail)
    else:
        L.call(base, dt, *head, _hip.ptr(ell), *tail)


def _split_grad_table(g, ell_shape, os_shape):
    ne = 1
    for s_ in ell_shape[1:]:
        ne *= s_
    return g[:, :ne].reshape(ell_shape), g[:, ne], (None if os_shape is None else g[:, ne + 1:].reshape(os_shape))


def factorize(kind, X, ell, oscale, noise, rhs, ws, Xs=None):
    L = _hip.lib()
    dt, dev = ws.dtype, ws.device
    st = _hip.stream_ptr(dev)
    k = kind_code(kind)
    q, n, d = ws.q, ws.n, X.shape[1]
    fused = os.environ.get("PLMC_FUSED_ASSEMBLE", "1") != "0"
    if not fused:
        _kernel_call(L, "plmc_assemble", dt, (k, _hip.ptr(X), n, d), ell, (_hip.ptr(oscale), _hip.ptr(noise),
                     _hip.ptr(ws.A), ws.lda, ws.strideA, q, st))
    nrhs = 0 if rhs is None else rhs.shape[1]
    if ws.naug_pad > 0:
        L.call("plmc_write_rhs", dt, _hip.ptr(rhs), nrhs, n, _hip.ptr(ws.A), ws.lda, ws.strideA, 0, ws.naug_pad, q, st)
    if Xs is not None:
        _kernel_call(L, "plmc_assemble_cross", dt, (k, _hip.ptr(X), n, _hip.ptr(Xs), Xs.shape[0], d), ell,
                     (_hip.ptr(oscale), _hip.ptr(ws.A), ws.lda, ws.strideA, ws.n_pad + nrhs, ws.n_pad, q, st))
    flags = (1 | (4 if ws.keep_planes else 0)) if ws.with_inverse else 0
    if fused:
        _kernel_call(L, "plmc_factorize_ex", dt, (k, _hip.ptr(X), n, d), ell, (_hip.ptr(oscale), _hip.ptr(noise), _hip.ptr(ws.A), ws.n_pad,
                     ws.lda, ws.naug, ws.strideA, _hip.ptr(ws.Vd), _hip.ptr(ws.logdet), _hip.ptr(ws.info), flags, q, _hip.ptr(noise), st))
    else:
        L.call("plmc_potrf_ex", dt, _hip.ptr(ws.A), ws.n_pad, ws.lda, ws.naug, ws.strideA, _hip.ptr(ws.Vd),
               _hip.ptr(ws.logdet), _hip.ptr(ws.info), flags, q, _hip.ptr(noise), st)


def factorize_checked(kind, X, ell, oscale, noise, rhs, ws, Xs=None):
    factorize(kind, X, ell, oscale, noise, rhs, ws, Xs)
    if not settings.check_cholesky.on():
        return 0.0
    check = PivotCheck.eager(ws)
    if not check.failed():
        return 0.0

    def attempt(jit):
        factorize(kind, X, ell, oscale, noise + jit, rhs, ws, Xs)
        return PivotCheck.eager(ws), None

    return walk(ws.dtype, check, attempt)[0]


class ExactLatentLogProb(torch.autograd.Function):

    @staticmethod
    def forward(ctx, X, ell, oscale, noise, y, kind, table=None):
        _hip.require_device(X, ell, noise, y)
        L = _hip.lib()
        dt, dev = y.dtype, y.device
        if dt not in (torch.float32, torch.float64):
            raise TypeError("projectedlmc hot path supports float32 and float64 tensors")
        q, n = y.shape
        d = X.shape[1]
        _check_kernel_shape(L, ell, kind)
        G = n_components(ell, kind)
        need_grad = any(ctx.needs_input_grad[1:5]) or table is not None
        Xc, ellc, osc, nzc, yc = (_contig(t, dt) for t in (X, ell, oscale, noise, y))
        ws = get_workspace(n, q, 1, dt, dev, need_grad, G, is_sm(ell), kind == PER)
        st = _hip.stream_ptr(dev)
        grad = table if table is not None else (torch.empty(q, grad_table_width(ell, kind), dtype=torch.float64, device=dev) if need_grad else None)
        check = settings.check_cholesky.on()

        def enqueue(noise_eff):
            factorize(kind, Xc, ellc, osc, noise_eff, yc.reshape(q, 1, n), ws)
            info = PivotCheck(ws) if check else None
            L.call("plmc_extract_col", dt, _hip.ptr(ws.A), ws.n_pad, ws.lda, ws.strideA, 0, _hip.ptr(ws.z),
                   _hip.ptr(ws.quad), q, st)
            if need_grad:
                L.call("plmc_wt_matvec", dt, _hip.ptr(ws.W), ws.n_pad, ws.ldw, ws.strideW, _hip.ptr(ws.z),
                       _hip.ptr(ws.alpha), q, st)
                gs = grad_stream(dev)
                gst = st
                if gs is not None:
                    gs.wait_stream(torch.cuda.current_stream(dev))
                    gst = _hip.stream_handle(gs, dev)
                    for t in (grad, Xc, ellc, osc, noise_eff):
                        if t is not None:
                            t.record_stream(gs)
                _kernel_call(L, "plmc_kinv_grad_vd", dt, (kind_code(kind), _hip.ptr(ws.W), ws.n_pad, ws.ldw, ws.strideW,
                             _hip.ptr(ws.alpha), _hip.ptr(Xc), n, d), ellc, (_hip.ptr(osc), _hip.ptr(grad),
                             None, 0, 0, None, _hip.ptr(ws.partials), q, _hip.ptr(noise_eff), _hip.ptr(ws.Vd), gst), stream=gs)
                if gs is not None:
                    ws.pending = torch.cuda.Event()
                    ws.pending.record(gs)
            lp = -0.5 * (ws.quad + ws.logdet + n * LOG2PI)
            return info, lp

        dc = deferred_pivot_checks.current if check else None
        if dc is not None:
            info, logp = enqueue(nzc + dc.jitter if dc.jitter > 0.0 else nzc)
            dc.pending.append(info)
        else:
            info, logp = enqueue(nzc)
            if check and info.failed():
                def attempt(jit):
                    nonlocal ws
                    ws = get_workspace(n, q, 1, dt, dev, need_grad, G, is_sm(ell), kind == PER)
                    return enqueue(nzc + jit)

                logp = walk(dt, info, attempt)[1]
        if need_grad:
            ctx.save_for_backward(grad, ws.alpha[:, :n].clone())
        ctx.grad_ready = getattr(ws, "pending", None) if need_grad else None
        ctx.ell_shape = ell.shape
        ctx.os_shape = None if oscale is None else oscale.shape
        ctx.table_out = table is not None
        return logp.to(dt)

    @staticmethod
    def backward(ctx, gout):
        grad, alpha = ctx.saved_tensors
        dt = alpha.dtype
        if ctx.table_out:
            return None, None, None, None, -(gout[:, None].to(dt) * alpha), None, None
        if ctx.grad_ready is not None:
            torch.cuda.current_stream(alpha.device).wait_event(ctx.grad_ready)
        g_ell, g_noise, g_os = _split_grad_table(gout.to(torch.float64)[:, None] * grad, ctx.ell_shape, ctx.os_shape)
        g_y = -(gout[:, None].to(dt) * alpha)
        return None, g_ell, g_os, g_noise, g_y, None, None


class _HyperGrad(torch.autograd.Function):

    @staticmethod
    def forward(ctx, ell, oscale, noise, table, zero):
        ctx.save_for_backward(table)
        ctx.ell_shape = ell.shape
        ctx.os_shape = None if oscale is None else oscale.shape
        return zero.detach()

    @staticmethod
    def backward(ctx, gout):
        (table,) = ctx.saved_tensors
        g = (table * gout[:, None]).to(gout.dtype)
        g_ell, g_noise, g_os = _split_grad_table(g, ctx.ell_shape, ctx.os_shape)
        return g_ell, g_os, g_noise, None, None


_zeros = {}


class HyperGradHandle:
    __slots__ = ("table", "hz")


def prepare_hyper_grad(ell, oscale, noise, kind=None):
    hyper = torch.is_grad_enabled() and any(t is not None and t.requires_grad for t in (ell, oscale, noise))
    gs = grad_stream(ell.device) if (hyper and ell.is_cuda) else None
    if gs is None:
        return None
    q = ell.shape[0]
    key = (ell.device.index, ell.dtype, q)
    zero = _zeros.get(key)
    if zero is None:
        zero = _zeros[key] = torch.zeros(q, dtype=ell.dtype, device=ell.device)
        torch.cuda.current_stream(ell.device).synchronize()
    h = HyperGradHandle()
    h.table = torch.empty(q, grad_table_width(ell, kind), dtype=torch.float64, device=ell.device)
    with torch.cuda.stream(gs):
        h.hz = _HyperGrad.apply(ell, oscale, noise, h.table, zero)
    return h


def exact_latent_log_prob(kind, X, ell, oscale, noise, y, hyper=None):
    if hyper is None:
        hyper = prepare_hyper_grad(ell, oscale, noise, kind)
    if hyper is None:
        return ExactLatentLogProb.apply(X, ell, oscale, noise, y, kind)
    det = lambda t: None if t is None else t.detach()
    lp = ExactLatentLogProb.apply(X, det(ell), det(oscale), det(noise), y, kind, hyper.table)
    return lp + hyper.hz


def exact_loo(kind, X, ell, oscale, noise, y):
    _hip.require_device(X, ell, noise, y)
    L = _hip.lib()
    dt, dev = y.dtype, y.device
    q, n = y.shape
    d = X.shape[1]
    Xc, ellc, osc, nzc, yc = (_contig(t, dt) for t in (X, ell, oscale, noise, y))
    _check_kernel_shape(L, ellc, kind)
    ws = get_workspace(n, q, 1, dt, dev, True, n_components(ellc, kind), is_sm(ellc), kind == PER)
    st = _hip.stream_ptr(dev)
    factorize_checked(kind, Xc, ellc, osc, nzc, yc.reshape(q, 1, n), ws)
    L.call("plmc_extract_col", dt, _hip.ptr(ws.A), ws.n_pad, ws.lda, ws.strideA, 0, _hip.ptr(ws.z),
           _hip.ptr(ws.quad), q, st)
    L.call("plmc_wt_matvec", dt, _hip.ptr(ws.W), ws.n_pad, ws.ldw, ws.strideW, _hip.ptr(ws.z),
           _hip.ptr(ws.alpha), q, st)
    grad = torch.empty(q, grad_table_width(ellc, kind), dtype=torch.float64, device=dev)
    kd = torch.empty(q, ws.n_pad, dtype=dt, device=dev)
    _kernel_call(L, "plmc_kinv_grad_vd", dt, (kind_code(kind), _hip.ptr(ws.W), ws.n_pad, ws.ldw, ws.strideW, _hip.ptr(ws.alpha),
                 _hip.ptr(Xc), n, d), ellc, (_hip.ptr(osc), _hip.ptr(grad), None, 0, 0, _hip.ptr(kd),
                 _hip.ptr(ws.partials), q, _hip.ptr(nzc), _hip.ptr(ws.Vd), st))
    sigma2 = 1.0 / kd[:, :n]
    return sigma2, ws.alpha[:, :n] * sigma2


class PosteriorCache:

    def __init__(self):
        self.key, self.ws = None, None
        self.seen = None
        self.hits = self.misses = 0

    def drop(self):
        self.key, self.ws = None, None
        self.seen = None


def model_state_key(module, *tensors):
    items = [(id(t), t._version) for t in list(module.parameters()) + list(module.buffers())]
    items += [(id(t), t._version, tuple(t.shape)) for t in tensors if t is not None]
    return tuple(items)


def exact_posterior(kind, X, ell, oscale, noise, y, Xs, full_cov=False, cache=None, key=None):
    _hip.require_device(X, ell, noise, y, Xs)
    L = _hip.lib()
    dt, dev = y.dtype, y.device
    q, n = y.shape
    ns = Xs.shape[0]
    Xc, Xsc, ellc, osc, nzc = (_contig(t, dt) for t in (X, Xs, ell, oscale, noise))
    _check_kernel_shape(L, ellc, kind)
    yc = _contig(y).reshape(q, 1, n)
    st = _hip.stream_ptr(dev)
    mode = settings.prediction_cache.value() if cache is not None else "off"
    hit = False
    if cache is not None and mode != "off":
        ws = cache.ws
        hit = (ws is not None and cache.key == key and key is not None and ws.dtype == dt and ws.device == dev and ws.n == n and ws.q == q
               and ws.naug >= 1 + ns)
    same_state = cache is not None and cache.ws is not None and key is not None and cache.key == key
    build = cache is not None and mode != "off" and not hit and (mode == "eager" or same_state or (key is not None and cache.seen == key))
    if not hit and not build:
        if cache is not None and mode != "off":
            cache.drop()
            cache.seen = key
            cache.misses += 1
        ws = get_workspace(n, q, 1 + ns, dt, dev, False)
        factorize_checked(kind, Xc, ellc, osc, nzc, yc, ws, Xs=Xsc)
    else:
        if hit:
            cache.hits += 1
            k = kind_code(kind)
            L.call("plmc_write_rhs", dt, _hip.ptr(yc), 1, n, _hip.ptr(ws.A), ws.lda, ws.strideA, 0, ws.naug_pad, q, st)
            _kernel_call(L, "plmc_assemble_cross", dt, (k, _hip.ptr(Xc), n, _hip.ptr(Xsc), ns, Xc.shape[1]), ellc, (_hip.ptr(osc),
                         _hip.ptr(ws.A), ws.lda, ws.strideA, ws.n_pad + 1, ws.n_pad, q, st))
            if ws.keep_planes:
                L.call("plmc_potrs_aug_kept", dt, _hip.ptr(ws.A), ws.n_pad, ws.lda, 1 + ns, ws.wcol0, ws.strideA, _hip.ptr(ws.Vd), q,
                       _hip.ptr(nzc), st)
            else:
                L.call("plmc_potrs_aug", dt, _hip.ptr(ws.A), ws.n_pad, ws.lda, 1 + ns, ws.wcol0, ws.strideA, _hip.ptr(ws.Vd), q, st)
        else:
            cache.misses += 1
            cache.drop()
            ws = Workspace(n, q, 1 + ns, dt, dev, with_inverse=True, keep_planes=True)
            factorize_checked(kind, Xc, ellc, osc, nzc, yc, ws, Xs=Xsc)
            cache.key, cache.ws = key, ws
    mean = torch.empty(q, ns, dtype=dt, device=dev)
    vsq = torch.empty(q, ns, dtype=dt, device=dev)
    L.call("plmc_posterior_moments", dt, _hip.ptr(ws.A), ws.n_pad, ws.lda, ws.strideA, ns, _hip.ptr(mean), _hip.ptr(vsq), q, st)
    if full_cov:
        V = ws.A[:, :, ws.n_pad + 1:ws.n_pad + 1 + ns]
        Kss = dense_cross(kind, Xsc, Xsc, ellc, osc)
        from ._dense import gemm_tn
        cov = Kss - gemm_tn(V, V)
        return mean, cov
    from .kernels import prior_diagonal
    var = prior_diagonal(kind, Xsc, osc, q) - vsq
    return mean, var


def mix_posterior(mean_lat, var_lat, Ht, eps=0.0):
    _hip.require_device(mean_lat, var_lat, Ht)
    L = _hip.lib()
    dt, dev = mean_lat.dtype, mean_lat.device
    q, ns = mean_lat.shape
    p = Ht.shape[1]
    ml, vl, H = (_contig(t, dt) for t in (mean_lat, var_lat, Ht))
    mean = torch.empty(ns, p, dtype=dt, device=dev)
    var = torch.empty(ns, p, dtype=dt, device=dev)
    L.call("plmc_mix_posterior", dt, _hip.ptr(ml), _hip.ptr(vl), _hip.ptr(H), q, ns, p, float(eps), _hip.ptr(mean), _hip.ptr(var),
           _hip.stream_ptr(dev))
    return mean, var


def dense_cross(kind, X1, X2, ell, oscale):
    L = _hip.lib()
    dt, dev = X1.dtype, X1.device
    q = ell.shape[0]
    n1, n2, d = X1.shape[0], X2.shape[0], X1.shape[1]
    out = torch.empty(q, n1, n2, dtype=dt, device=dev)
    _kernel_call(L, "plmc_assemble_cross", dt, (kind_code(kind), _hip.ptr(X1.contiguous()), n1, _hip.ptr(X2.contiguous()), n2, d),
                 ell.contiguous(), (_hip.ptr(None if oscale is None else oscale.contiguous()), _hip.ptr(out),
                 n2, n1 * n2, 0, n1, q, _hip.stream_ptr(dev)))
    return out
```

projected-lmc_amd/projectedlmc/_hip.py:

```python
import ctypes
import os

import torch

_HERE = os.path.dirname(os.path.abspath(__file__))
LIB_PATH = os.environ.get("PLMC_LIB") or os.path.join(_HERE, "libplmc_hip.so")

ABI_VERSION = 4
KIND = {"rbf": 0, "matern12": 1, "matern32": 2, "matern52": 3, "spline": 4}

_c = ctypes
_P = _c.c_void_p
_I = _c.c_int
_L = _c.c_int64

_TYPED = {
    "plmc_assemble": [_I, _P, _I, _I, _P, _P, _P, _P, _L, _L, _I, _P],
    "plmc_assemble_add": [_I, _P, _I, _I, _I, _P, _P, _P, _P, _L, _L, _I, _P],
    "plmc_assemble_per": [_P, _I, _I, _P, _P, _P, _P, _P, _L, _L, _I, _P],
    "plmc_assemble_sm": [_P, _I, _I, _I, _P, _P, _P, _P, _P, _L, _L, _I, _P],
    "plmc_write_rhs": [_P, _I, _I, _P, _L, _L, _I, _I, _I, _P],
    "plmc_assemble_cross": [_I, _P, _I, _P, _I, _I, _P, _P, _P, _L, _L, _L, _L, _I, _P],
    "plmc_assemble_cross_add": [_I, _P, _I, _P, _I, _I, _I, _P, _P, _P, _L, _L, _L, _L, _I, _P],
    "plmc_assemble_cross_per": [_P, _I, _P, _I, _I, _P, _P, _P, _P, _L, _L, _L, _L, _I, _P],
    "plmc_assemble_cross_sm": [_P, _I, _P, _I, _I, _I, _P, _P, _P, _P, _L, _L, _L, _L, _I, _P],
    "plmc_potrf": [_P, _L, _L, _I, _L, _P, _P, _P, _I, _I, _P],
    "plmc_potrf_ex": [_P, _L, _L, _I, _L, _P, _P, _P, _I, _I, _P, _P],
    "plmc_factorize_ex": [_I, _P, _I, _I, _P, _P, _P, _P, _L, _L, _I, _L, _P, _P, _P, _I, _I, _P, _P],
    "plmc_factorize_add_ex": [_I, _P, _I, _I, _I, _P, _P, _P, _P, _L, _L, _I, _L, _P, _P, _P, _I, _I, _P, _P],
    "plmc_factorize_per_ex": [_P, _I, _I, _P, _P, _P, _P, _P, _L, _L, _I, _L, _P, _P, _P, _I, _I, _P, _P],
    "plmc_factorize_sm_ex": [_P, _I, _I, _I, _P, _P, _P, _P, _P, _L, _L, _I, _L, _P, _P, _P, _I, _I, _P, _P],
    "plmc_potrs_aug": [_P, _L, _L, _I, _L, _L, _P, _I, _P],
    "plmc_potrs_aug_kept": [_P, _L, _L, _I, _L, _L, _P, _I, _P, _P],
    "plmc_extract_col": [_P, _L, _L, _L, _I, _P, _P, _I, _P],
    "plmc_wt_matvec": [_P, _L, _L, _L, _P, _P, _I, _P],
    "plmc_w_diag": [_P, _L, _L, _L, _P, _I, _P],
    "plmc_gemm_tn": [_I, _I, _I, _I, _P, _L, _L, _P, _L, _L, _P, _L, _L, _I, _P],
    "plmc_gemm_tn_tri": [_I, _I, _I, _I, _I, _P, _L, _L, _P, _L, _L, _P, _L, _L, _I, _P],
    "plmc_kinv_grad": [_I, _P, _L, _L, _L, _P, _P, _I, _I, _P, _P, _P, _P, _L, _L, _P, _P, _I, _P],
    "plmc_kinv_grad_ex": [_I, _P, _L, _L, _L, _P, _P, _I, _I, _P, _P, _P, _P, _L, _L, _P, _P, _I, _P, _P],
    "plmc_kinv_grad_vd": [_I, _P, _L, _L, _L, _P, _P, _I, _I, _P, _P, _P, _P, _L, _L, _P, _P, _I, _P, _P, _P],
    "plmc_kinv_grad_add_vd": [_I, _P, _L, _L, _L, _P, _P, _I, _I, _I, _P, _P, _P, _P, _L, _L, _P, _P, _I, _P, _P, _P],
    "plmc_kinv_grad_per_vd": [_P, _L, _L, _L, _P, _P, _I, _I, _P, _P, _P, _P, _P, _L, _L, _P, _P, _I, _P, _P, _P],
    "plmc_kinv_grad_sm_vd": [_P, _L, _L, _L, _P, _P, _I, _I, _I, _P, _P, _P, _P, _P, _L, _L, _P, _P, _I, _P, _P, _P],
    "plmc_lmc_assemble": [_I, _P, _I, _I, _I, _I, _P, _P, _P, _P, _P, _L, _P],
    "plmc_lmc_cross": [_I, _P, _I, _P, _I, _I, _I, _I, _P, _P, _P, _P, _L, _L, _L, _P],
    "plmc_lmc_kinv_grad": [_I, _P, _L, _L, _P, _P, _I, _I, _I, _I, _P, _P, _P, _P, _P, _P],
    "plmc_kernel_vjp": [_I, _P, _I, _P, _I, _I, _P, _P, _P, _L, _L, _P, _P, _P, _I, _P],
    "plmc_kernel_vjp_add": [_I, _P, _I, _P, _I, _I, _I, _P, _P, _P, _L, _L, _P, _P, _P, _I, _P],
    "plmc_qr_small": [_P, _I, _I, _L, _P, _L, _P, _L, _P],
    "plmc_comm_allreduce_sum": [_P, _L, _P],
    "plmc_posterior_moments": [_P, _L, _L, _L, _I, _P, _P, _I, _P],
    "plmc_mix_posterior": [_P, _P, _P, _I, _I, _I, _c.c_double, _P, _P, _P],
}
_PLAIN = {
    "plmc_version": ([], _I),
    "plmc_block": ([], _I),
    "plmc_pad": ([_L], _L),
    "plmc_vd_blocks": ([_L, _L], _L),
    "plmc_vd_blocks_for": ([_L, _L, _I], _L),
    "plmc_vd_blocks_keep": ([_L, _L], _L),
    "plmc_split_scales_offset": ([_L, _L], _L),
    "plmc_max_dim": ([], _I),
    "plmc_max_components": ([], _I),
    "plmc_sm_max_mixtures": ([], _I),
    "plmc_sm_max_dim": ([], _I),
    "plmc_sm_grad_partials_bytes": ([_L, _I, _I, _I], _L),
    "plmc_per_max_dim": ([], _I),
    "plmc_per_grad_partials_bytes": ([_L, _I, _I], _L),
    "plmc_qr_max": ([], _I),
    "plmc_last_error": ([], _c.c_char_p),
    "plmc_grad_scratch_bytes": ([_L, _I], _L),
    "plmc_grad_scratch_bytes_for": ([_L, _I, _I], _L),
    "plmc_grad_partials_bytes": ([_L, _I], _L),
    "plmc_lmc_grad_len": ([_I, _I, _I], _L),
    "plmc_lmc_grad_scratch_bytes": ([_L, _I, _I, _I], _L),
    "plmc_prof_enable": ([_I], _I),
    "plmc_prof_kernels": ([], _I),
    "plmc_prof_name": ([_I], _c.c_char_p),
    "plmc_prof_collect": ([_P, _P, _P, _P], _I),
    "plmc_prof_mfma_rate": ([_I, _P, _L, _P], _I),
    "plmc_dev_reload_knobs": ([], _I),
    "plmc_comm_unique_id": ([_P], _I),
    "plmc_comm_init": ([_P, _I, _I], _I),
    "plmc_comm_world": ([], _I),
    "plmc_comm_rank": ([], _I),
    "plmc_comm_destroy": ([], _I),
}


def prof_enable(on):
    L = lib().cdll
    if isinstance(on, (list, tuple, set)):
        names = [L.plmc_prof_name(i).decode() for i in range(L.plmc_prof_kernels())]
        mask = 0
        for k in on:
            mask |= 1 << names.index(k)
        return L.plmc_prof_enable(mask << 1)
    return L.plmc_prof_enable(1 if on else 0)


def prof_collect():
    L = lib().cdll
    k = L.plmc_prof_kernels()
    ms, fl, by = (_c.c_double * k)(), (_c.c_double * k)(), (_c.c_double * k)()
    la = (_c.c_int64 * k)()
    L.plmc_prof_collect(ms, la, fl, by)
    return {L.plmc_prof_name(i).decode(): dict(ms=ms[i], launches=la[i], flops=fl[i], bytes=by[i])
            for i in range(k) if la[i] > 0}


class knob:

    def __init__(self, name, value):
        self.name, self.value = name, value

    def __enter__(self):
        self.old = os.environ.get(self.name)
        os.environ[self.name] = str(self.value)
        lib().cdll.plmc_dev_reload_knobs()
        return self

    def __exit__(self, *exc):
        if self.old is None:
            os.environ.pop(self.name, None)
        else:
            os.environ[self.name] = self.old
        lib().cdll.plmc_dev_reload_knobs()
        return False


def mfma_rate(dtype=torch.float32, device=None):
    L = lib().cdll
    dev = torch.device("cuda", torch.cuda.current_device()) if device is None else device
    kind = 2 if dtype == "bf16" else int(dtype == torch.float64)
    sink = torch.empty(4 * 1024 * 256, dtype=torch.float32 if kind == 2 else dtype, device=dev)
    out = _c.c_double(0.0)
    with torch.cuda.device(dev):
        torch.cuda.synchronize(dev)
        rc = L.plmc_prof_mfma_rate(kind, ptr(sink), sink.numel() * sink.element_size(), _c.byref(out))
    if rc != 0:
        raise RuntimeError("plmc_prof_mfma_rate failed: %s" % L.plmc_last_error().decode())
    return out.value


def exported_symbols():
    names = list(_PLAIN)
    for base in _TYPED:
        names += [base + "_f32", base + "_f64"]
    return names


class _Lib:
    def __init__(self):
        if not os.path.exists(LIB_PATH):
            raise RuntimeError(
                "projectedlmc: %s not found -- build it with `python -c 'import __graft_entry__ as g; g.build()'` "
                "(hipcc --offload-arch=gfx950).  There is no CPU fallback." % LIB_PATH)
        self.cdll = ctypes.CDLL(LIB_PATH)
        for name, (args, res) in _PLAIN.items():
            fn = getattr(self.cdll, name)
            fn.argtypes, fn.restype = args, res
        for base, args in _TYPED.items():
            for suf in ("_f32", "_f64"):
                fn = getattr(self.cdll, base + suf)
                fn.argtypes, fn.restype = args, _I
        if self.cdll.plmc_version() != ABI_VERSION:
            raise RuntimeError("projectedlmc: %s is ABI version %d, this package needs %d (the scratch-size contract of "
                               "plmc_potrf_* / plmc_kinv_grad_* differs) -- rebuild it" % (LIB_PATH, self.cdll.plmc_version(), ABI_VERSION))

    def call(self, base, dtype, *args):
        suf = "_f32" if dtype == torch.float32 else "_f64"
        fn = getattr(self.cdll, base + suf)
        device = next((a.device for a in reversed(args) if isinstance(a, StreamHandle)), None)
        if device is not None and device.index is not None and device.index != torch.cuda.current_device():
            with torch.cuda.device(device):
                rc = fn(*args)
        else:
            rc = fn(*args)
        if rc != 0:
            raise RuntimeError("%s%s failed (%d): %s" % (base, suf, rc, self.cdll.plmc_last_error().decode()))


_lib = None


def lib():
    global _lib
    if _lib is None:
        _lib = _Lib()
    return _lib


def ptr(t):
    return None if t is None else _c.c_void_p(t.data_ptr())


class StreamHandle(_c.c_void_p):
    device = None


def stream_handle(stream, device):
    h = StreamHandle(stream.cuda_stream)
    h.device = torch.device(device) if not isinstance(device, torch.device) else device
    if h.device.index is None:
        h.device = torch.device("cuda", torch.cuda.current_device())
    return h


def stream_ptr(device):
    return stream_handle(torch.cuda.current_stream(device), device)


def require_device(*tensors):
    for t in tensors:
        if t is not None and not t.is_cuda:
            raise RuntimeError(
                "projectedlmc (MI355X build): the exact-GP hot path runs only on ROCm device tensors "
                "(got a %s tensor); there is no CPU fallback -- move model and data with .cuda()." % t.device.type)
```

Measured before the change: 56.91 iters/sec.

## Split kinv-grad into alpha-free and alpha-only passes overlapped on streams

Splits the fused K^-1/alpha gradient kernel into a Kinv-only pass, which can start on the grad stream right after factorization without waiting for the alpha solve, and a separate alpha-outer-product pass on the main stream. Each pass writes its own partials set, and a last-block atomic counter reduces both sets into the gradient in-kernel, replacing the separate reduce launch. The point is to overlap gradient work with extract_col/wt_matvec and drop a launch. In exchange it adds a second pass over tile geometry, more kernel-evaluation work, and atomic-counter synchronisation.

```diff
diff --git a/include/plmc.h b/include/plmc.h
--- a/include/plmc.h
+++ b/include/plmc.h
@@ -22,6 +22,7 @@
 int64_t     plmc_grad_scratch_bytes_for(int64_t n_pad, int q, int elem_bytes);
 int64_t     plmc_grad_scratch_bytes(int64_t n_pad, int q);
 int64_t     plmc_grad_partials_bytes(int64_t n_pad, int q);
+int64_t     plmc_grad_split_partials_bytes(int64_t n_pad, int q);
 
 int plmc_assemble_f32(int kind, const float *X, int n, int d, const float *ell, const float *oscale,
                       const float *noise, float *A, int64_t lda, int64_t strideA, int q, void *stream);
@@ -126,6 +127,16 @@
                           const double *alpha, const double *X, int n, int d, const double *ell,
                           const double *oscale, double *grad, double *Kinv, int64_t ldk, int64_t strideK,
                           double *kinv_diag, void *partials, int q, const double *eig_lo, const double *Vd, void *stream);
+int plmc_kinv_grad_split_vd_f32(int kind, const float *W, int64_t n_pad, int64_t ldw, int64_t strideW,
+                                const float *alpha, const float *X, int n, int d, const float *ell,
+                                const float *oscale, double *grad, float *Kinv, int64_t ldk, int64_t strideK,
+                                float *kinv_diag, void *partials, int q, const float *eig_lo, const float *Vd,
+                                void *alpha_stream, void *stream);
+int plmc_kinv_grad_split_vd_f64(int kind, const double *W, int64_t n_pad, int64_t ldw, int64_t strideW,
+                                const double *alpha, const double *X, int n, int d, const double *ell,
+                                const double *oscale, double *grad, double *Kinv, int64_t ldk, int64_t strideK,
+                                double *kinv_diag, void *partials, int q, const double *eig_lo, const double *Vd,
+                                void *alpha_stream, void *stream);
 
 int plmc_max_components(void);
 int plmc_assemble_add_f32(int kind, const float *X, int n, int d, int ncomp, const float *ell, const float *oscale,
diff --git a/projected-lmc_amd/csrc/api.hip b/projected-lmc_amd/csrc/api.hip
--- a/projected-lmc_amd/csrc/api.hip
+++ b/projected-lmc_amd/csrc/api.hip
@@ -45,6 +45,7 @@
   g_knobs.chain = getenv("PLMC_CHAIN") ? atoi(getenv("PLMC_CHAIN")) : 1;
   g_knobs.chain_nw = getenv("PLMC_CHAIN_NW") ? atoi(getenv("PLMC_CHAIN_NW")) : 0;
   g_knobs.chain_edge = getenv("PLMC_CHAIN_EDGE") ? atoi(getenv("PLMC_CHAIN_EDGE")) : 0;
+  g_knobs.alpha_fused = getenv("PLMC_ALPHA_FUSED") && atoi(getenv("PLMC_ALPHA_FUSED")) != 0;
   g_knobs_loaded = true;
 }
 const Knobs &knobs() {
diff --git a/projected-lmc_amd/csrc/api_common.hpp b/projected-lmc_amd/csrc/api_common.hpp
--- a/projected-lmc_amd/csrc/api_common.hpp
+++ b/projected-lmc_amd/csrc/api_common.hpp
@@ -54,6 +54,7 @@
   int chain;
   int chain_edge;
   int chain_nw;
+  bool alpha_fused;
 };
 const Knobs &knobs();
 
@@ -94,6 +95,8 @@
 
 hipStream_t side_stream(int which = 0);
 hipEvent_t sync_event(int idx);
+void api_lock();
+void api_unlock();
 void bind_sweep_ctx(hipStream_t caller, int e_prev_idx);
 
 inline bool aligned16(const void *p) { return (reinterpret_cast<uintptr_t>(p) & 15) == 0; }
diff --git a/projected-lmc_amd/csrc/kinv_epilogue.inc b/projected-lmc_amd/csrc/kinv_epilogue.inc
--- a/projected-lmc_amd/csrc/kinv_epilogue.inc
+++ b/projected-lmc_amd/csrc/kinv_epilogue.inc
@@ -23,14 +23,14 @@
       smem[L::UI + r * L::LDI + k] = (k < d && gi < n) ? X[(int64_t)gi * d + k] * inv : T(0);
       smem[L::UJ + r * L::LDI + k] = (k < d && gj < n) ? X[(int64_t)gj * d + k] * inv : T(0);
     }
-    if (tid < NB) {
+    if (AMODE != AM_KINV && tid < NB) {
       smem[L::AI + tid] = live ? alpha[(int64_t)lat * n_pad + ib * NB + tid] : T(0);
       smem[L::AJ + tid] = live ? alpha[(int64_t)lat * n_pad + jb * NB + tid] : T(0);
     }
     __syncthreads();
     const bool interior = ib < jb && (jb + 1) * NB <= n && !Kinv && !kinv_diag;
 #define PLMC_GRAD_TILE(KIND, INT) \
-  grad_tile_small<T, DCAP, KIND, INT>(acc, smem, tid, os, ib, jb, n, lat, n_pad, Kinv, ldk, strideK, kinv_diag, g, g_noise, g_os)
+  grad_tile_small<T, DCAP, KIND, INT, AMODE>(acc, smem, tid, os, ib, jb, n, lat, n_pad, Kinv, ldk, strideK, kinv_diag, g, g_noise, g_os)
     if (interior) {
       if (kind == K_RBF) PLMC_GRAD_TILE(K_RBF, true);
       else if (kind == K_MATERN12) PLMC_GRAD_TILE(K_MATERN12, true);
@@ -71,7 +71,7 @@
     ui[r * ldu + k] = gi < n ? X[(int64_t)gi * d + k] * inv : T(0);
     uj[r * ldu + k] = gj < n ? X[(int64_t)gj * d + k] * inv : T(0);
   }
-  if (tid < NB) {
+  if (AMODE != AM_KINV && tid < NB) {
     ai[tid] = live ? alpha[(int64_t)lat * n_pad + ib * NB + tid] : T(0);
     aj[tid] = live ? alpha[(int64_t)lat * n_pad + jb * NB + tid] : T(0);
   }
@@ -95,19 +95,26 @@
 #pragma unroll
             for (int k = 0; k < DCAP; ++k) xi[k] = k < d ? uir[k] : T(0);
           }
-          const T a_i = ai[row];
+          T a_i = T(0);
+          if constexpr (AMODE != AM_KINV) a_i = ai[row];
 #pragma unroll
           for (int nt = 0; nt < 4; ++nt) {
             const int col = tile_col(wn, nt, lane);
             const int gj = jb * NB + col;
-            const auto &av = acc.v[mt][nt];
-            const T kin = r == 0 ? av[0] : (r == 1 ? av[1] : (r == 2 ? av[2] : av[3]));
-            if (first) {
+            T kin = T(0);
+            if constexpr (AMODE != AM_ALPHA) {
+              const auto &av = acc.v[mt][nt];
+              kin = r == 0 ? av[0] : (r == 1 ? av[1] : (r == 2 ? av[2] : av[3]));
+            }
+            if (AMODE != AM_ALPHA && first) {
               if (Kinv && gj >= gi) Kinv[(int64_t)lat * strideK + (int64_t)gi * ldk + gj] = kin;
               if (kinv_diag && gi == gj) kinv_diag[(int64_t)lat * n_pad + gi] = kin;
             }
             if (gi < n && gj < n && gj >= gi) {
-              const T wij = a_i * aj[col] - kin;
+              T wij;
+              if constexpr (AMODE == AM_KINV) wij = -kin;
+              else if constexpr (AMODE == AM_ALPHA) wij = a_i * aj[col];
+              else wij = a_i * aj[col] - kin;
               const T *ujc = uj + col * ldu;
               T df2[KD];
               T r2 = T(0);
diff --git a/projected-lmc_amd/csrc/potri_grad.hip b/projected-lmc_amd/csrc/potri_grad.hip
--- a/projected-lmc_amd/csrc/potri_grad.hip
+++ b/projected-lmc_amd/csrc/potri_grad.hip
@@ -9,12 +9,14 @@
 
 constexpr int GP = MAX_DIM + 2;
 
+enum AlphaMode { AM_FUSED = 0, AM_KINV = 1, AM_ALPHA = 2 };
+
 template <int DCAP> struct GradLds {
   static constexpr int LDI = DCAP + 4;
   static constexpr int UI = 0, UJ = UI + NB * LDI, AI = UJ + NB * LDI, AJ = AI + NB, ACCS = AJ + NB, END = ACCS + 4 * NTHREADS * 4;
 };
 
-template <typename T, int DCAP, int KIND, bool INTERIOR>
+template <typename T, int DCAP, int KIND, bool INTERIOR, int AMODE = AM_FUSED>
 __device__ __forceinline__ void grad_tile_small(const Acc<T> &acc, T *smem, const int tid, T os, int ib, int jb, int n, int lat, int64_t n_pad,
                                                 T *Kinv, int64_t ldk, int64_t strideK, T *kinv_diag, T (&g)[DCAP],
                                                 T &g_noise, T &g_os) {
@@ -33,7 +35,9 @@
 #define PLMC_PARK(M)                                                                                    \
   _Pragma("unroll") for (int nt = 0; nt < 4; ++nt) _Pragma("unroll") for (int r = 0; r < 4; ++r)         \
       accs[nt * NTHREADS * 4 + r] = acc.v[M][nt][r];
-    if (mt == 0) { PLMC_PARK(0) } else if (mt == 1) { PLMC_PARK(1) } else if (mt == 2) { PLMC_PARK(2) } else { PLMC_PARK(3) }
+    if constexpr (AMODE != AM_ALPHA) {
+      if (mt == 0) { PLMC_PARK(0) } else if (mt == 1) { PLMC_PARK(1) } else if (mt == 2) { PLMC_PARK(2) } else { PLMC_PARK(3) }
+    }
 #undef PLMC_PARK
 #pragma unroll 1
     for (int nt = 0; nt < 4; ++nt) {
@@ -42,12 +46,14 @@
       T2 u2[NP];
 #pragma unroll
       for (int j = 0; j < NP; ++j) u2[j] = *reinterpret_cast<const T2 *>(ujc + 2 * j);
-      const T a_j = smem[L::AJ + col];
+      T a_j = T(0);
+      if constexpr (AMODE != AM_KINV) a_j = smem[L::AJ + col];
       const int gj = jb * NB + col;
 #pragma unroll 1
       for (int r = 0; r < 4; ++r) {
         const int row = tile_row<T>(wm, mt, lane, r);
-        const T kin = accs[nt * NTHREADS * 4 + r];
+        T kin = T(0);
+        if constexpr (AMODE != AM_ALPHA) kin = accs[nt * NTHREADS * 4 + r];
         const T *uir = smem + L::UI + row * L::LDI;
         T2 df[NP];
         T2 r2p = {T(0), T(0)};
@@ -68,7 +74,10 @@
         } else {
           kern_value_base_fast(KIND, r2p.x + r2p.y, val, base);
         }
-        T w = smem[L::AI + row] * a_j - kin;
+        T w;
+        if constexpr (AMODE == AM_KINV) w = -kin;
+        else if constexpr (AMODE == AM_ALPHA) w = smem[L::AI + row] * a_j;
+        else w = smem[L::AI + row] * a_j - kin;
         if (!INTERIOR) {
           const int gi = ib * NB + row;
           if (Kinv && gj >= gi) Kinv[(int64_t)lat * strideK + (int64_t)gi * ldk + gj] = kin;
@@ -96,7 +105,7 @@
 
 template <typename T, int DCAP> constexpr int KG_MIN_WAVES = sizeof(T) == 8 ? 2 : (DCAP <= 8 ? 4 : (DCAP <= 16 ? 2 : 1));
 
-template <typename T, int DCAP, bool SPLINE>
+template <typename T, int DCAP, bool SPLINE, int AMODE>
 __device__ __forceinline__ void kinv_tile_epilogue(const Acc<T> &acc, T *smem, const int tid, const bool live, int kind, int ib, int jb, int lat,
                                                    int m, int64_t n_pad, const T *__restrict__ alpha, const T *__restrict__ X, int n, int d,
                                                    const T *__restrict__ ell, const T *__restrict__ oscale, T *Kinv, int64_t ldk,
@@ -118,19 +127,116 @@
   acc.zero();                                                                                                                                  \
   tile_mainloop<T, false, true>(acc, Wl + (int64_t)ib * NB, ldw, Wl + (int64_t)jb * NB, ldw, (int)(n_pad - (int64_t)jb * NB), smem)
 
-template <typename T, int DCAP, bool SPLINE = false>
+constexpr int FIN_NT = 256, FIN_U = 4;
+typedef double f64x2 __attribute__((ext_vector_type(2)));
+template <typename T, int DCAP>
+__device__ __forceinline__ void grad_finish(unsigned *counter, int expect, const double *partials, int m, int d, int nlat, int lat,
+                                            const T *__restrict__ ell, double *__restrict__ grad, double *lds) {
+  constexpr int NPAIR = DCAP / 2 + 1, NG = FIN_NT / NPAIR;
+  static_assert(DCAP % 2 == 0 && MAX_DIM % 2 == 0 && GP % 2 == 0, "16-byte loads of slot pairs");
+  asm volatile("s_waitcnt vmcnt(0)" ::: "memory");
+  __syncthreads();
+  int *flag = reinterpret_cast<int *>(lds);
+  if (threadIdx.x == 0) {
+    __builtin_amdgcn_fence(__ATOMIC_RELEASE, "agent");
+    asm volatile("s_waitcnt vmcnt(0)" ::: "memory");
+    const unsigned t = __hip_atomic_fetch_add(counter + lat, 1u, __ATOMIC_RELAXED, __HIP_MEMORY_SCOPE_AGENT);
+    const int last = t == (unsigned)(expect - 1);
+    if (last) {
+      __builtin_amdgcn_fence(__ATOMIC_ACQUIRE, "agent");
+      asm volatile("s_waitcnt vmcnt(0)" ::: "memory");
+    }
+    *flag = last;
+  }
+  __syncthreads();
+  const int last = *flag;
+  __syncthreads();
+  if (!last) return;
+  const int t = threadIdx.x;
+  const int mm = m * m, nt = m * (m + 1) / 2;
+  f64x2 tot = {0.0, 0.0};
+  if (t < NG * NPAIR) {
+    const int p = t % NPAIR, grp = t / NPAIR;
+    const int slot0 = p < DCAP / 2 ? 2 * p : MAX_DIM;
+    const double *b0 = partials + (int64_t)lat * mm * GP + slot0;
+    const double *b1 = b0 + (int64_t)nlat * mm * GP;
+    f64x2 s[FIN_U];
+#pragma unroll
+    for (int u = 0; u < FIN_U; ++u) s[u] = f64x2{0.0, 0.0};
+    for (int r0 = grp; r0 < 2 * nt; r0 += FIN_U * NG) {
+      f64x2 v[FIN_U];
+#pragma unroll
+      for (int u = 0; u < FIN_U; ++u) {
+        const int r = r0 + u * NG;
+        const int rc = r < 2 * nt ? r : 0;
+        const int set = rc >= nt ? 1 : 0;
+        int ib, jb;
+        tri_decode(rc - set * nt, ib, jb);
+        v[u] = *reinterpret_cast<const f64x2 *>((set ? b1 : b0) + (int64_t)(ib * m + jb) * GP);
+      }
+#pragma unroll
+      for (int u = 0; u < FIN_U; ++u) s[u] += r0 + u * NG < 2 * nt ? v[u] : f64x2{0.0, 0.0};
+    }
+    tot = (s[0] + s[1]) + (s[2] + s[3]);
+  }
+  f64x2 *red = reinterpret_cast<f64x2 *>(lds);
+  if (t < FIN_NT) red[t] = tot;
+  __syncthreads();
+  if (t < NPAIR) {
+    f64x2 a = {0.0, 0.0};
+    for (int g = 0; g < NG; ++g) a += red[g * NPAIR + t];
+    double *gl = grad + (int64_t)lat * (d + 2);
+    if (t < DCAP / 2) {
+      if (2 * t < d) gl[2 * t] = 0.5 * a.x / (double)ell[(int64_t)lat * d + 2 * t];
+      if (2 * t + 1 < d) gl[2 * t + 1] = 0.5 * a.y / (double)ell[(int64_t)lat * d + 2 * t + 1];
+    } else {
+      gl[d] = 0.5 * a.x;
+      gl[d + 1] = 0.5 * a.y;
+    }
+  }
+}
+
+template <typename T, int DCAP, bool SPLINE = false, int AMODE = AM_FUSED>
 __global__ __launch_bounds__(NTHREADS, (KG_MIN_WAVES<T, DCAP>)) void k_kinv_grad(int kind, const T *__restrict__ W, int64_t n_pad, int64_t ldw,
                                                          int64_t strideW, const T *__restrict__ alpha,
                                                          const T *__restrict__ X, int n, int d,
                                                          const T *__restrict__ ell, const T *__restrict__ oscale,
                                                          T *Kinv, int64_t ldk, int64_t strideK, T *kinv_diag,
-                                                         double *__restrict__ partials, int nlat) {
+                                                         double *__restrict__ partials, int nlat, unsigned *counter, int expect,
+                                                         double *__restrict__ grad) {
   PLMC_KINV_TILE_PRODUCT;
   const int tid = threadIdx.x;
   constexpr bool live = true;
 #define PLMC_KINV_KEEP (sizeof(T) == 4)
 #include "kinv_epilogue.inc"
 #undef PLMC_KINV_KEEP
+  if constexpr (AMODE == AM_KINV) grad_finish<T, DCAP>(counter, expect, partials, m, d, nlat, lat, ell, grad, reinterpret_cast<double *>(smem));
+}
+
+template <typename T, int DCAP> constexpr int alpha_smem_elems() {
+  return DCAP <= 8 ? GradLds<DCAP>::ACCS : 2 * NB * (MAX_DIM + 1) + 2 * NB + 4 * GP * (int)(sizeof(double) / sizeof(T));
+}
+template <typename T, int DCAP, bool SPLINE = false>
+__global__ __launch_bounds__(NTHREADS) void k_alpha_grad(int kind, int64_t n_pad, const T *__restrict__ alpha, const T *__restrict__ X, int n, int d,
+                                                         const T *__restrict__ ell, const T *__restrict__ oscale, double *__restrict__ partials,
+                                                         int nlat, unsigned *counter, int expect, double *__restrict__ grad,
+                                                         const double *partials0) {
+  constexpr int AMODE = AM_ALPHA;
+  static_assert(alpha_smem_elems<T, DCAP>() * sizeof(T) >= FIN_NT * 16 && alpha_smem_elems<T, DCAP>() * sizeof(T) >= 4 * GP * sizeof(double), "LDS of the sums");
+  const int m = (int)(n_pad / NB);
+  const int lat = (int)blockIdx.x % nlat;
+  int ib, jb;
+  tri_decode((int)blockIdx.x / nlat, ib, jb);
+  __shared__ __align__(16) T smem[alpha_smem_elems<T, DCAP>()];
+  const Acc<T> acc = {};
+  T *const Kinv = nullptr, *const kinv_diag = nullptr;
+  constexpr int64_t ldk = 0, strideK = 0;
+  const int tid = threadIdx.x;
+  constexpr bool live = true;
+#define PLMC_KINV_KEEP (sizeof(T) == 4)
+#include "kinv_epilogue.inc"
+#undef PLMC_KINV_KEEP
+  grad_finish<T, DCAP>(counter, expect, partials0, m, d, nlat, lat, ell, grad, reinterpret_cast<double *>(smem));
 }
 
 #define PLMC_KINV_BF3_TILE_PRODUCT                                                                                                             \
@@ -161,15 +267,17 @@
   const int half = __builtin_amdgcn_readfirstlane((int)threadIdx.x >> 8);                                                                      \
   const int ib = ibm + half
 
-template <class S, int DCAP, bool SPLINE = false>
+template <class S, int DCAP, bool SPLINE = false, int AMODE = AM_FUSED>
 __global__ __launch_bounds__(B3_NT, 2) void k_kinv_grad_bf3(int kind, int64_t n_pad, const float *__restrict__ alpha, const float *__restrict__ X, int n,
                                                             int d, const float *__restrict__ ell, const float *__restrict__ oscale, float *Kinv,
                                                             int64_t ldk, int64_t strideK, float *kinv_diag, double *__restrict__ partials, int nlat,
                                                             const unsigned short *__restrict__ Wp, const float *__restrict__ wscale,
-                                                            int64_t wp_lat_stride, int64_t ws_stride) {
+                                                            int64_t wp_lat_stride, int64_t ws_stride, unsigned *counter, int expect,
+                                                            double *__restrict__ grad) {
   PLMC_KINV_BF3_TILE_PRODUCT;
-  kinv_tile_epilogue<float, DCAP, SPLINE>(acc0, reinterpret_cast<float *>(lds) + half * tile_smem_elems<float>(), (int)threadIdx.x & 255, ib <= jb, kind,
-                                          ib, jb, lat, m, n_pad, alpha, X, n, d, ell, oscale, Kinv, ldk, strideK, kinv_diag, partials);
+  kinv_tile_epilogue<float, DCAP, SPLINE, AMODE>(acc0, reinterpret_cast<float *>(lds) + half * tile_smem_elems<float>(), (int)threadIdx.x & 255, ib <= jb,
+                                                 kind, ib, jb, lat, m, n_pad, alpha, X, n, d, ell, oscale, Kinv, ldk, strideK, kinv_diag, partials);
+  if constexpr (AMODE == AM_KINV) grad_finish<float, DCAP>(counter, expect, partials, m, d, nlat, lat, ell, grad, reinterpret_cast<double *>(lds));
 }
 
 
@@ -313,10 +421,12 @@
   }
 }
 
+struct AlphaSplit { hipStream_t alpha_st; };
+
 template <typename T, class S>
 int kinv_grad_impl(const CovTable &table, const T *W, int64_t n_pad, int64_t ldw, int64_t strideW, const T *alpha, const T *X, int n, double *grad,
                    T *Kinv, int64_t ldk, int64_t strideK, T *kinv_diag, void *partials, int q, const float *eig_lo, void *stream,
-                   const float *Vd = nullptr, int64_t lda_vd = 0) {
+                   const float *Vd = nullptr, int64_t lda_vd = 0, const AlphaSplit *as = nullptr) {
   PLMC_REQUIRE_TABLE(table);
   const CovFamily family = table.route();
   const int kind = table.kind, d = table.d, ncomp = table.ncomp, rows = table.partials_rows();
@@ -331,6 +441,49 @@
   const int m = (int)(n_pad / NB);
   double *part = reinterpret_cast<double *>(partials);
   const double np = (double)n_pad;
+  bool split_alpha = as && as->alpha_st != st && family == COV_PLAIN && !knobs().alpha_fused && aligned16(partials);
+  double *part1 = part + (int64_t)m * m * q * GP;
+  unsigned *counter = reinterpret_cast<unsigned *>(part1 + (int64_t)m * m * q * GP);
+  int expect = m * (m + 1);
+  auto alpha_order = [&]() -> int {
+    if (!as || as->alpha_st == st) return 0;
+    api_lock();
+    bind_sweep_ctx(as->alpha_st, 8);
+    hipStream_t side = split_alpha ? side_stream() : nullptr;
+    hipEvent_t e_zero = sync_event(13), e_alpha = sync_event(14);
+    api_unlock();
+    if (!e_zero || !e_alpha) return fail("plmc_kinv_grad_split_vd", "no ordering event");
+    (void)hipEventRecord(e_alpha, as->alpha_st);
+    if (!split_alpha || !side) {
+      split_alpha = false;
+      (void)hipStreamWaitEvent(st, e_alpha, 0);
+      return 0;
+    }
+    (void)hipMemsetAsync(counter, 0, (size_t)q * sizeof(unsigned), st);
+    (void)hipEventRecord(e_zero, st);
+    (void)hipStreamWaitEvent(side, e_zero, 0);
+    (void)hipStreamWaitEvent(side, e_alpha, 0);
+    return 0;
+  };
+  auto alpha_launch = [&]() -> int {
+    api_lock();
+    hipStream_t side = side_stream();
+    hipEvent_t e_done = sync_event(15);
+    api_unlock();
+    if (!e_done) return fail("plmc_kinv_grad_split_vd", "no ordering event");
+    const dim3 grid(q * (m * (m + 1) / 2)), block(NTHREADS);
+#define PLMC_LAUNCH_AG(DC, SP) \
+  hipLaunchKernelGGL((k_alpha_grad<T, DC, SP>), grid, block, 0, side, kind, n_pad, alpha, X, n, d, ell, oscale, part1, q, counter, expect, grad, \
+                     (const double *)part)
+    if (d <= 4) PLMC_LAUNCH_AG(4, false);
+    else if (d <= 8) PLMC_LAUNCH_AG(8, false);
+    else if (d <= 16) { if (kind == K_SPLINE) PLMC_LAUNCH_AG(16, true); else PLMC_LAUNCH_AG(16, false); }
+    else { if (kind == K_SPLINE) PLMC_LAUNCH_AG(32, true); else PLMC_LAUNCH_AG(32, false); }
+#undef PLMC_LAUNCH_AG
+    (void)hipEventRecord(e_done, side);
+    (void)hipStreamWaitEvent(st, e_done, 0);
+    return 0;
+  };
   if constexpr (!std::is_void<S>::value) {
     PLMC_REQUIRE(q <= 1024, "too many latents for one scale launch");
     const unsigned short *wp = nullptr;
@@ -350,12 +503,23 @@
       wsc = wsco;
       wp_lat = b3_elems<S>(n_pad, n_pad);
       ws_lat = 1;
+      split_alpha = false;
+    }
+    if (alpha_order() != 0) return -1;
+    {
+      int live = 0;
+      for (int jb = 0; jb < m; ++jb) live += jb / 2 + 1;
+      expect = live + m * (m + 1) / 2;
     }
     const int SJ = (m + 7) / 8, NSB = SJ * (SJ + 1) / 2;
     const dim3 gridb(8 * ((q * NSB + 7) / 8) * 32);
-#define PLMC_LAUNCH_KB(DC, SP) \
-  hipLaunchKernelGGL((k_kinv_grad_bf3<S, DC, SP>), gridb, dim3(B3_NT), 0, st, kind, n_pad, alpha, X, n, d, ell, oscale, Kinv, ldk, strideK, kinv_diag, \
-                     part, q, wp, wsc, wp_lat, ws_lat)
+#define PLMC_LAUNCH_KB(DC, SP)                                                                                                                            \
+  if (split_alpha)                                                                                                                                        \
+    hipLaunchKernelGGL((k_kinv_grad_bf3<S, DC, SP, AM_KINV>), gridb, dim3(B3_NT), 0, st, kind, n_pad, alpha, X, n, d, ell, oscale, Kinv, ldk, strideK,    \
+                       kinv_diag, part, q, wp, wsc, wp_lat, ws_lat, counter, expect, grad);                                                               \
+  else                                                                                                                                                    \
+    hipLaunchKernelGGL((k_kinv_grad_bf3<S, DC, SP, AM_FUSED>), gridb, dim3(B3_NT), 0, st, kind, n_pad, alpha, X, n, d, ell, oscale, Kinv, ldk, strideK,   \
+                       kinv_diag, part, q, wp, wsc, wp_lat, ws_lat, (unsigned *)nullptr, 0, (double *)nullptr)
 #define PLMC_LAUNCH_TB(F, DC) \
   hipLaunchKernelGGL((k_kinv_grad_add_bf3<S, F, DC>), gridb, dim3(B3_NT), 0, st, kind, ncomp, n_pad, alpha, X, n, d, ell, oscale, Kinv, ldk, strideK, \
                      kinv_diag, part, q, wp, wsc, wp_lat, ws_lat, (const float *)second)
@@ -365,18 +529,23 @@
       case COV_SM: PLMC_LAUNCH_TB(COV_SM, 1); break;
       case COV_ADD: PLMC_LAUNCH_TB(COV_ADD, 0); break;
       case COV_PLAIN:
-        if (d <= 4) PLMC_LAUNCH_KB(4, false);
-        else if (d <= 8) PLMC_LAUNCH_KB(8, false);
-        else if (d <= 16) { if (kind == K_SPLINE) PLMC_LAUNCH_KB(16, true); else PLMC_LAUNCH_KB(16, false); }
-        else { if (kind == K_SPLINE) PLMC_LAUNCH_KB(32, true); else PLMC_LAUNCH_KB(32, false); }
+        if (d <= 4) { PLMC_LAUNCH_KB(4, false); }
+        else if (d <= 8) { PLMC_LAUNCH_KB(8, false); }
+        else if (d <= 16) { if (kind == K_SPLINE) { PLMC_LAUNCH_KB(16, true); } else { PLMC_LAUNCH_KB(16, false); } }
+        else { if (kind == K_SPLINE) { PLMC_LAUNCH_KB(32, true); } else { PLMC_LAUNCH_KB(32, false); } }
     }
 #undef PLMC_LAUNCH_TB
 #undef PLMC_LAUNCH_KB
   } else {
+    if (alpha_order() != 0) return -1;
     const dim3 grid(q * (m * (m + 1) / 2)), block(NTHREADS);
-#define PLMC_LAUNCH_KG(DC, SP)                                                                                       \
-  hipLaunchKernelGGL((k_kinv_grad<T, DC, SP>), grid, block, 0, st, kind, W, n_pad, ldw, strideW, alpha, X, n, d, ell, \
-                     oscale, Kinv, ldk, strideK, kinv_diag, part, q)
+#define PLMC_LAUNCH_KG(DC, SP)                                                                                                     \
+  if (split_alpha)                                                                                                                 \
+    hipLaunchKernelGGL((k_kinv_grad<T, DC, SP, AM_KINV>), grid, block, 0, st, kind, W, n_pad, ldw, strideW, alpha, X, n, d, ell,   \
+                       oscale, Kinv, ldk, strideK, kinv_diag, part, q, counter, expect, grad);                                     \
+  else                                                                                                                             \
+    hipLaunchKernelGGL((k_kinv_grad<T, DC, SP, AM_FUSED>), grid, block, 0, st, kind, W, n_pad, ldw, strideW, alpha, X, n, d, ell,  \
+                       oscale, Kinv, ldk, strideK, kinv_diag, part, q, (unsigned *)nullptr, 0, (double *)nullptr)
 #define PLMC_LAUNCH_TG(F, DC) \
   hipLaunchKernelGGL((k_kinv_grad_add<T, F, DC>), grid, block, 0, st, kind, ncomp, W, n_pad, ldw, strideW, alpha, X, n, d, ell, oscale, Kinv, ldk, \
                      strideK, kinv_diag, part, q, second)
@@ -386,15 +555,17 @@
       case COV_SM: if (d == 1) PLMC_LAUNCH_TG(COV_SM, 1); else if (d <= 4) PLMC_LAUNCH_TG(COV_SM, 4); else PLMC_LAUNCH_TG(COV_SM, 8); break;
       case COV_ADD: PLMC_LAUNCH_TG(COV_ADD, 0); break;
       case COV_PLAIN:
-        if (d <= 4) PLMC_LAUNCH_KG(4, false);
-        else if (d <= 8) PLMC_LAUNCH_KG(8, false);
-        else if (d <= 16) { if (kind == K_SPLINE) PLMC_LAUNCH_KG(16, true); else PLMC_LAUNCH_KG(16, false); }
-        else { if (kind == K_SPLINE) PLMC_LAUNCH_KG(32, true); else PLMC_LAUNCH_KG(32, false); }
+        if (d <= 4) { PLMC_LAUNCH_KG(4, false); }
+        else if (d <= 8) { PLMC_LAUNCH_KG(8, false); }
+        else if (d <= 16) { if (kind == K_SPLINE) { PLMC_LAUNCH_KG(16, true); } else { PLMC_LAUNCH_KG(16, false); } }
+        else { if (kind == K_SPLINE) { PLMC_LAUNCH_KG(32, true); } else { PLMC_LAUNCH_KG(32, false); } }
     }
 #undef PLMC_LAUNCH_TG
 #undef PLMC_LAUNCH_KG
   }
-  {
+  if (split_alpha) {
+    if (alpha_launch() != 0) return -1;
+  } else {
     ProfScope ps(PK_REDUCE, st, 0.0, (double)m * m * q * rows * GP * sizeof(double) / 2);
     switch (family) {
       case COV_PER: hipLaunchKernelGGL(k_reduce_grad_per<T>, dim3(q), dim3(RED_NT), 0, st, part, m, d, ell, second, grad); break;
@@ -419,22 +590,27 @@
   const int64_t m = n_pad / plmc::NB;
   return m * m * (int64_t)q * plmc::GP * (int64_t)sizeof(double);
 }
+int64_t plmc_grad_split_partials_bytes(int64_t n_pad, int q) {
+  return 2 * plmc_grad_partials_bytes(n_pad, q) + ((int64_t)q * (int64_t)sizeof(unsigned) + 255) / 256 * 256;
+}
 static int kinv_grad_f32_any(const plmc::CovTable &table, const float *W, int64_t n_pad, int64_t ldw, int64_t strideW, const float *alpha,
                              const float *X, int n, double *grad, float *Kinv, int64_t ldk, int64_t strideK, float *kinv_diag, void *partials, int q,
-                             const float *eig_lo, void *stream, const float *Vd = nullptr) {
+                             const float *eig_lo, void *stream, const float *Vd = nullptr, const plmc::AlphaSplit *as = nullptr) {
   const int split = plmc::knobs().split;
   if (split == 0 || ((table.family == plmc::COV_SM || table.family == plmc::COV_PER) && table.d > 1))
-    return plmc::kinv_grad_impl<float, void>(table, W, n_pad, ldw, strideW, alpha, X, n, grad, Kinv, ldk, strideK, kinv_diag, partials, q, nullptr, stream);
+    return plmc::kinv_grad_impl<float, void>(table, W, n_pad, ldw, strideW, alpha, X, n, grad, Kinv, ldk, strideK, kinv_diag, partials, q, nullptr, stream,
+                                             nullptr, 0, as);
   if (split == 2 && eig_lo)
     return plmc::kinv_grad_impl<float, plmc::SplitH2>(table, W, n_pad, ldw, strideW, alpha, X, n, grad, Kinv, ldk, strideK, kinv_diag, partials, q, eig_lo,
-                                                      stream, Vd, ldw);
+                                                      stream, Vd, ldw, as);
   return plmc::kinv_grad_impl<float, plmc::SplitB3>(table, W, n_pad, ldw, strideW, alpha, X, n, grad, Kinv, ldk, strideK, kinv_diag, partials, q, nullptr,
-                                                    stream, Vd, ldw);
+                                                    stream, Vd, ldw, as);
 }
 static int kinv_grad_f64(const plmc::CovTable &table, const double *W, int64_t n_pad, int64_t ldw, int64_t strideW, const double *alpha,
                          const double *X, int n, double *grad, double *Kinv, int64_t ldk, int64_t strideK, double *kinv_diag, void *partials, int q,
-                         void *stream) {
-  return plmc::kinv_grad_impl<double, void>(table, W, n_pad, ldw, strideW, alpha, X, n, grad, Kinv, ldk, strideK, kinv_diag, partials, q, nullptr, stream);
+                         void *stream, const plmc::AlphaSplit *as = nullptr) {
+  return plmc::kinv_grad_impl<double, void>(table, W, n_pad, ldw, strideW, alpha, X, n, grad, Kinv, ldk, strideK, kinv_diag, partials, q, nullptr, stream,
+                                            nullptr, 0, as);
 }
 using plmc::CovTable;
 int plmc_kinv_grad_f32(int kind, const float *W, int64_t n_pad, int64_t ldw, int64_t strideW, const float *alpha,
@@ -465,6 +641,24 @@
   (void)eig_lo;
   (void)Vd;
   return kinv_grad_f64(CovTable::plain(kind, d, ell, oscale), W, n_pad, ldw, strideW, alpha, X, n, grad, Kinv, ldk, strideK, kinv_diag, partials, q, stream);
+}
+int plmc_kinv_grad_split_vd_f32(int kind, const float *W, int64_t n_pad, int64_t ldw, int64_t strideW, const float *alpha,
+                                const float *X, int n, int d, const float *ell, const float *oscale, double *grad,
+                                float *Kinv, int64_t ldk, int64_t strideK, float *kinv_diag, void *partials, int q,
+                                const float *eig_lo, const float *Vd, void *alpha_stream, void *stream) {
+  const plmc::AlphaSplit as{(hipStream_t)alpha_stream};
+  return kinv_grad_f32_any(CovTable::plain(kind, d, ell, oscale), W, n_pad, ldw, strideW, alpha, X, n, grad, Kinv, ldk, strideK, kinv_diag, partials, q,
+                           eig_lo, stream, Vd, &as);
+}
+int plmc_kinv_grad_split_vd_f64(int kind, const double *W, int64_t n_pad, int64_t ldw, int64_t strideW, const double *alpha,
+                                const double *X, int n, int d, const double *ell, const double *oscale, double *grad,
+                                double *Kinv, int64_t ldk, int64_t strideK, double *kinv_diag, void *partials, int q,
+                                const double *eig_lo, const double *Vd, void *alpha_stream, void *stream) {
+  (void)eig_lo;
+  (void)Vd;
+  const plmc::AlphaSplit as{(hipStream_t)alpha_stream};
+  return kinv_grad_f64(CovTable::plain(kind, d, ell, oscale), W, n_pad, ldw, strideW, alpha, X, n, grad, Kinv, ldk, strideK, kinv_diag, partials, q, stream,
+                       &as);
 }
 int plmc_kinv_grad_add_vd_f32(int kind, const float *W, int64_t n_pad, int64_t ldw, int64_t strideW, const float *alpha,
                               const float *X, int n, int d, int ncomp, const float *ell, const float *oscale, double *grad,
diff --git a/projected-lmc_amd/projectedlmc/_engine.py b/projected-lmc_amd/projectedlmc/_engine.py
--- a/projected-lmc_amd/projectedlmc/_engine.py
+++ b/projected-lmc_amd/projectedlmc/_engine.py
@@ -42,6 +42,7 @@
             self.alpha = torch.empty(q, self.n_pad, dtype=dtype, device=device)
             nbytes = int(L.cdll.plmc_sm_grad_partials_bytes(self.n_pad, q, ncomp, esz) if sm
                          else L.cdll.plmc_per_grad_partials_bytes(self.n_pad, q, esz) if per
+                         else L.cdll.plmc_grad_split_partials_bytes(self.n_pad, q) if ncomp == 1
                          else L.cdll.plmc_grad_partials_bytes(self.n_pad, q * ncomp))
             self.partials = torch.empty(nbytes // 8, dtype=torch.float64, device=device)
 
@@ -240,23 +241,32 @@
 
         def enqueue(noise_eff):
             factorize(kind, Xc, ellc, osc, noise_eff, yc.reshape(q, 1, n), ws)
+            gs = grad_stream(dev) if need_grad else None
+            alpha_free = gs is not None and ellc.dim() == 2 and kind != PER
+            if alpha_free:
+                gs.wait_stream(torch.cuda.current_stream(dev))
             info = PivotCheck(ws) if check else None
             L.call("plmc_extract_col", dt, _hip.ptr(ws.A), ws.n_pad, ws.lda, ws.strideA, 0, _hip.ptr(ws.z),
                    _hip.ptr(ws.quad), q, st)
             if need_grad:
                 L.call("plmc_wt_matvec", dt, _hip.ptr(ws.W), ws.n_pad, ws.ldw, ws.strideW, _hip.ptr(ws.z),
                        _hip.ptr(ws.alpha), q, st)
-                gs = grad_stream(dev)
                 gst = st
                 if gs is not None:
-                    gs.wait_stream(torch.cuda.current_stream(dev))
+                    if not alpha_free:
+                        gs.wait_stream(torch.cuda.current_stream(dev))
                     gst = _hip.stream_handle(gs, dev)
                     for t in (grad, Xc, ellc, osc, noise_eff):
                         if t is not None:
                             t.record_stream(gs)
-                _kernel_call(L, "plmc_kinv_grad_vd", dt, (kind_code(kind), _hip.ptr(ws.W), ws.n_pad, ws.ldw, ws.strideW,
-                             _hip.ptr(ws.alpha), _hip.ptr(Xc), n, d), ellc, (_hip.ptr(osc), _hip.ptr(grad),
-                             None, 0, 0, None, _hip.ptr(ws.partials), q, _hip.ptr(noise_eff), _hip.ptr(ws.Vd), gst), stream=gs)
+                if alpha_free:
+                    L.call("plmc_kinv_grad_split_vd", dt, kind_code(kind), _hip.ptr(ws.W), ws.n_pad, ws.ldw, ws.strideW,
+                           _hip.ptr(ws.alpha), _hip.ptr(Xc), n, d, _hip.ptr(ellc), _hip.ptr(osc), _hip.ptr(grad),
+                           None, 0, 0, None, _hip.ptr(ws.partials), q, _hip.ptr(noise_eff), _hip.ptr(ws.Vd), st, gst)
+                else:
+                    _kernel_call(L, "plmc_kinv_grad_vd", dt, (kind_code(kind), _hip.ptr(ws.W), ws.n_pad, ws.ldw, ws.strideW,
+                                 _hip.ptr(ws.alpha), _hip.ptr(Xc), n, d), ellc, (_hip.ptr(osc), _hip.ptr(grad),
+                                 None, 0, 0, None, _hip.ptr(ws.partials), q, _hip.ptr(noise_eff), _hip.ptr(ws.Vd), gst), stream=gs)
                 if gs is not None:
                     ws.pending = torch.cuda.Event()
                     ws.pending.record(gs)
diff --git a/projected-lmc_amd/projectedlmc/_hip.py b/projected-lmc_amd/projectedlmc/_hip.py
--- a/projected-lmc_amd/projectedlmc/_hip.py
+++ b/projected-lmc_amd/projectedlmc/_hip.py
@@ -40,6 +40,7 @@
     "plmc_kinv_grad": [_I, _P, _L, _L, _L, _P, _P, _I, _I, _P, _P, _P, _P, _L, _L, _P, _P, _I, _P],
     "plmc_kinv_grad_ex": [_I, _P, _L, _L, _L, _P, _P, _I, _I, _P, _P, _P, _P, _L, _L, _P, _P, _I, _P, _P],
     "plmc_kinv_grad_vd": [_I, _P, _L, _L, _L, _P, _P, _I, _I, _P, _P, _P, _P, _L, _L, _P, _P, _I, _P, _P, _P],
+    "plmc_kinv_grad_split_vd": [_I, _P, _L, _L, _L, _P, _P, _I, _I, _P, _P, _P, _P, _L, _L, _P, _P, _I, _P, _P, _P, _P],
     "plmc_kinv_grad_add_vd": [_I, _P, _L, _L, _L, _P, _P, _I, _I, _I, _P, _P, _P, _P, _L, _L, _P, _P, _I, _P, _P, _P],
     "plmc_kinv_grad_per_vd": [_P, _L, _L, _L, _P, _P, _I, _I, _P, _P, _P, _P, _P, _L, _L, _P, _P, _I, _P, _P, _P],
     "plmc_kinv_grad_sm_vd": [_P, _L, _L, _L, _P, _P, _I, _I, _I, _P, _P, _P, _P, _P, _L, _L, _P, _P, _I, _P, _P, _P],
@@ -73,6 +74,7 @@
     "plmc_grad_scratch_bytes": ([_L, _I], _L),
     "plmc_grad_scratch_bytes_for": ([_L, _I, _I], _L),
     "plmc_grad_partials_bytes": ([_L, _I], _L),
+    "plmc_grad_split_partials_bytes": ([_L, _I], _L),
     "plmc_lmc_grad_len": ([_I, _I, _I], _L),
     "plmc_lmc_grad_scratch_bytes": ([_L, _I, _I, _I], _L),
     "plmc_prof_enable": ([_I], _I),
```

Result: slower. 56.08 iters/sec (-1.5%).
